# Zain-Jiang/Speech-Editing-Toolkit

Hardware: AMD Instinct MI355X
Metric: diffusion mel-frames/s (100-step p_sample, B=32/GPU, T=800) (higher is better)
Workload: dtype f32 (operands carried as 2 fp16 pieces, 3 MFMA products per term, fp32 accumulate: fp32-equivalent, see roofline.note)

## Files before the change

### include/set_amd.h

```cpp
#ifndef SET_AMD_H
#define SET_AMD_H

#include <stdint.h>

#ifdef __cplusplus
extern "C" {
#endif

#define SET_AMD_ABI_VERSION 5

#define SET_OK 0
#define SET_E_INVALID (-1)
#define SET_E_UNSUPPORTED (-2)
#define SET_E_LAUNCH (-3)

#define SET_ACT_NONE 0
#define SET_ACT_RELU 1
#define SET_ACT_GELU 2
#define SET_ACT_TANH 3
#define SET_ACT_SOFTPLUS 4
#define SET_ACT_MISH 5
#define SET_ACT_LRELU 6

#define SET_PRO_NONE 0
#define SET_PRO_LRELU 1
#define SET_PRO_DIV 2

#define SET_IMPL_NAIVE 1
#define SET_IMPL_MFMA 2
#define SET_IMPL_MFMA2 3

#define SET_IMPL_BF16 4
#define SET_IMPL_F16X2 5

#define SET_IMPL_FEWOUT 6

#define SET_DTYPE_F32 0
#define SET_DTYPE_BF16 1
#define SET_DTYPE_BF16_G16 2
#define SET_DTYPE_BF16_G16_X16 3

int set_abi_version(void);
const char *set_last_error(void);

typedef struct SetConv1dArgs {
    const float *in;
    const float *w;
    const float *bias;
    const float *res;
    const float *mask;
    const float *in_chan_add;
    float *out;
    int64_t in_bs, in_cs, out_bs, out_cs, res_bs, res_cs;
    int64_t w_base, w_sco, w_sci, w_stap;
    int32_t B, Cin, Cout, K, dil, pad;
    int32_t T_in, T_iter, T_out, out_stride, out_off;
    int32_t pro, act, accumulate, impl;
    float pro_param, act_param, alpha;
    float out_div;
} SetConv1dArgs;

int set_conv1d(const SetConv1dArgs *args, void *stream);

int64_t set_packed_conv_weight_size(int32_t Cout, int32_t Cin, int32_t K);
int set_pack_conv_weight(const float *w, float *wp, int32_t Cout, int32_t Cin, int32_t K,
                         int64_t w_base, int64_t w_sco, int64_t w_sci, int64_t w_stap, void *stream);

int64_t set_packed_conv_weight_x2_size(int32_t Cout, int32_t Cin, int32_t K);
int set_pack_conv_weight_x2(const float *w, void *wp, int32_t Cout, int32_t Cin, int32_t K, int64_t w_base, int64_t w_sco,
                            int64_t w_sci, int64_t w_stap, int32_t scale_exp, void *stream);
int64_t set_packed_conv_transpose_x2_size(int32_t Cout, int32_t Cin, int32_t k, int32_t u);
int set_pack_conv_transpose_x2(const float *w, void *wp, int32_t Cout, int32_t Cin, int32_t k, int32_t u, int32_t scale_exp,
                               void *stream);
int set_conv_transpose1d_x2(const float *in, const void *wp, const float *bias, float *out, int32_t B, int32_t Cin, int32_t Cout,
                            int32_t k, int32_t u, int32_t P, int32_t T_in, int32_t pro, float pro_param, void *stream);
int set_conv_x2_range_flag(int32_t *flag, int32_t reset);

typedef struct SetResblockPairArgs {
    const float *x;
    const void *w1;
    const float *b1;
    const void *w2;
    const float *b2;
    float *out;
    int64_t x_bs, x_cs, out_bs, out_cs;
    int32_t B, C, K, dil, T;
    int32_t accumulate;
    float slope, out_div;
} SetResblockPairArgs;
int64_t set_sizeof_resblock_pair_args(void);
int set_resblock_pair_x2_supported(int32_t C, int32_t K, int32_t dil, int32_t T);
int set_resblock_pair_x2(const SetResblockPairArgs *args, void *stream);

int64_t set_packed_conv_weight_v2_size(int32_t Cout, int32_t Cin, int32_t K);
int set_pack_conv_weight_v2(const float *w, float *wp, int32_t Cout, int32_t Cin, int32_t K, int32_t dil,
                            int64_t w_base, int64_t w_sco, int64_t w_sci, int64_t w_stap, void *stream);

int set_weight_norm_fold(const float *g, const float *v, float *w, int32_t n0, int64_t inner, void *stream);

int set_layernorm_ch(const float *x, const float *gamma, const float *beta, const float *mask, float *out,
                     int32_t B, int32_t C, int32_t T, float eps, void *stream);
int set_embedding_bct(const int64_t *idx, const float *table, float *out, int32_t B, int32_t T, int32_t C,
                      int32_t n_rows, float scale, int32_t accumulate, void *stream);
int set_embedding_bct_dev_scale(const int64_t *idx, const float *table, float *out, int32_t B, int32_t T, int32_t C,
                                int32_t n_rows, const float *scale_dev, int32_t accumulate, void *stream);
int set_abs_sum_mask(const float *x, float *mask, int32_t B, int32_t C, int32_t T, void *stream);
int set_index_mask(const int64_t *idx, float *mask, int64_t n, void *stream);
int set_expand_states(const float *enc, const int64_t *mel2ph, float *out, int32_t B, int32_t C,
                      int32_t T_txt, int32_t T, void *stream);
int set_add_chan_mask(const float *x, const float *add, const float *mask, float *out, int32_t B, int32_t C,
                      int32_t T, void *stream);
int set_masked_dur(const int64_t *mel2ph, const float *tmask, const int64_t *txt, int64_t *out, int32_t B,
                   int32_t T, int32_t T_txt, void *stream);
int set_pitch_coarse(const float *f0_in, const float *uv_in, const float *tmask, const int64_t *mel2ph_pad,
                     int32_t uv_from_logit, float *f0_denorm, int64_t *coarse, int64_t n, void *stream);
int set_transpose_btc_to_bct(const float *in, float *out, int32_t B, int32_t T, int32_t C, void *stream);
int set_transpose_bct_to_btc(const float *in, float *out, int32_t B, int32_t C, int32_t T, void *stream);
int set_sum_scale(const float *a, const float *b, const float *c, float *out, float div, int64_t n, void *stream);
int set_blend_mask(const float *a, const float *b, const float *m, float *out, int64_t n, int64_t inner, void *stream);
int set_mul_one_minus_mask(const float *x, const float *m, float *out, int64_t n, int64_t inner, void *stream);
int set_dur_total(const float *dur, const int64_t *txt, int64_t *total, int32_t B, int32_t T_txt, void *stream);
int set_length_regulate(const float *dur, const int64_t *txt, int64_t *mel2ph, int32_t B, int32_t T_txt,
                        int32_t T_out, void *stream);

int set_sinusoid_embed(const float *t, float *out, int32_t dim, int32_t n, void *stream);

int set_gate(const float *y, float *z, int32_t B, int32_t C, int32_t T, void *stream);
int set_res_skip(const float *x_in, const float *o, float *x_out, float *skip, int32_t B, int32_t C, int32_t T,
                 int32_t first, void *stream);

typedef struct SetDiffnetLayerArgs {
    const float *x_in;
    const float *condproj;
    const float *dstep;
    const float *w1p;
    const float *b_dil;
    const float *w2p;
    const float *b_out;
    float *x_out;
    float *skip;
    int64_t cp_bs, d_bs, d_cs;
    int32_t B, T, dil, first;
    uint64_t *dbg_clock;
} SetDiffnetLayerArgs;
int set_diffnet_layer(const SetDiffnetLayerArgs *args, void *stream);
int64_t set_diffnet_w1p_size(void);
int64_t set_diffnet_w2p_size(void);
int set_pack_diffnet_layer(const float *w_dil, const float *w_out, float *w1p, float *w2p, void *stream);
int set_pack_diffnet_layers(const float *w_dil, const float *w_out, int64_t wd_ls, int64_t wo_ls, float *w1p, float *w2p,
                            float *w1w, float *w2w, int32_t L, void *stream);

typedef struct SetDiffnetStackArgs {
    float *xa, *xb, *skip;
    const float *condproj;
    const float *dstep;
    const float *w1p_all;
    const float *w2p_all;
    const float *b_dil_all;
    const float *b_out_all;
    int32_t *sync_ws;
    int64_t cp_bs, cp_ls, d_bs, d_cs, d_ls;
    int32_t B, T, L, dilation_cycle_length;
    const float *w1w_all;
    const float *w2w_all;
    float *x_all;
    float *save_y;
    float *save_z;
    int32_t *err_flag;
    const float *w1s_all;
    const float *w2s_all;
    float *z_ws;
    const void *wx3_all;
    int32_t x3_mode;
} SetDiffnetStackArgs;
int set_diffnet_stack(const SetDiffnetStackArgs *args, void *stream);
int64_t set_sizeof_diffnet_stack_args(void);

int64_t set_diffnet_layer_x3_image_size(int32_t mode);
int set_pack_diffnet_layer_x3(const float *w_dil , const float *w_out , void *img, int32_t mode,
                              int32_t k1, int32_t k2, void *stream);
int set_diffnet_stack_variant(int B, int T, int dilation_cycle_length, int images);
int set_diffnet_stack_x3_winograd(int B, int T, int dilation_cycle_length, int images);
int64_t set_diffnet_w1w_size(void);
int set_pack_diffnet_layer_wino(const float *w_dil, const float *w_out, float *w1w, float *w2w, void *stream);

int set_posterior_step(const float *x0, const float *x_t, const float *eps, const float *coef4, int64_t coef_bs,
                       float *x_prev, int32_t B, int64_t per_batch, uint64_t seed, uint64_t offset, void *stream);
int set_q_sample(const float *x_start, const float *eps, const float *ab2, const float *nonpad, float *x_t,
                 int32_t B, int32_t M, int32_t T, void *stream);
int set_randn(float *out, int64_t n, uint64_t seed, uint64_t offset, void *stream);
int set_rng_seed_delta(const uint64_t *dev_word);
int set_stream_order(void *first, void *after, int32_t slot);
int set_stream_mark(void *stream, int32_t slot, int32_t dev);
int set_stream_mark_done(int32_t slot);
int set_stream_create_low_priority(void **out);

typedef struct SetDiffLoopArgs {
    int32_t B, T, M, L, steps, dilation_cycle_length;
    float *x;
    const float *noise;
    uint64_t seed;
    const float *condproj;
    const float *dstep;
    const float *coef4;
    const float *w_in_p;
    const float *b_in;
    const float *w1p_all;
    const float *w2p_all;
    const float *b_dil_all;
    const float *b_out_all;
    const float *w1w_all;
    const float *w2w_all;
    const float *w1s_all;
    const float *w2s_all;
    float *z_ws;
    const void *wx3_all;
    int32_t x3_mode;
    const void *w_skip_x2, *w_outp_x2, *w_in_x2;
    const float *w_skip_p;
    const float *b_skip;
    const float *w_outp_p;
    const float *b_outp;
    float *ws_x0, *ws_x1, *ws_skip, *ws_h;
    float *ws_x0pred;
    float *layer_span_ms;
    float *loop_ms;
    int32_t n_groups;
    int32_t persistent;
    int32_t *sync_ws;
    int32_t *err_flag;
    const float *cond;
    const void *img16_all;
    const float *b_cond_all;
    float *bf16_ws;
    int64_t bf16_ws_floats;
} SetDiffLoopArgs;
int set_diffusion_loop(const SetDiffLoopArgs *args, void *stream);

int set_conv1d_wgrad(const float *g, const float *x, const float *chan_add, float *dw, int32_t B, int32_t Cin,
                     int32_t Cout, int32_t K, int32_t dil, int32_t pad, int32_t T, int32_t T_in, int32_t pro,
                     float pro_param, int32_t impl, void *stream);

int64_t set_conv1d_wgrad_scratch_floats(int32_t B, int32_t Cin, int32_t Cout, int32_t K, int32_t T, int32_t dtype);
int set_conv1d_wgrad_det(const void *g, const void *x, const float *chan_add, float *dw, int32_t B, int32_t Cin,
                         int32_t Cout, int32_t K, int32_t dil, int32_t pad, int32_t T, int32_t T_in, int32_t pro,
                         float pro_param, int32_t dtype, float *scratch, int64_t scratch_floats, void *stream);
int64_t set_conv1d_wgrad_grouped_scratch_floats(int32_t groups, int32_t B, int32_t Cin, int32_t Cout, int32_t K, int32_t T);
int set_conv1d_wgrad_det_grouped(const void *g, const void *x, const float *chan_add, float *dw, int32_t groups, int64_t g_gs,
                                 int64_t x_gs, int64_t add_gs, int64_t dw_gs, int32_t B, int32_t Cin, int32_t Cout, int32_t K,
                                 int32_t dil, int32_t pad, int32_t T, int32_t T_in, int32_t dtype, float *scratch,
                                 int64_t scratch_floats, void *stream);

typedef struct SetDiffnetLayerBf16Args {
    const float *x_in;
    float *x_out;
    float *skip;
    const float *cond;
    const float *dstep;
    const void *img;
    const float *b_dil, *b_cond, *b_out;
    uint16_t *y16;
    uint16_t *z16;
    int64_t d_bs, d_cs;
    int32_t B, T, dil, first;
} SetDiffnetLayerBf16Args;
int64_t set_sizeof_diffnet_layer_bf16_args(void);
int64_t set_diffnet_layer_bf16_image_size(void);
int set_pack_diffnet_layer_bf16(const float *wdil , const float *wcond ,
                                const float *wout , void *img, void *stream);
int set_pack_diffnet_layers_bf16(const float *wdil, const float *wcond, const float *wout, int64_t sdil, int64_t scond, int64_t sout,
                                 void *img, int32_t L, void *stream);
int set_diffnet_layer_fwd_bf16(const SetDiffnetLayerBf16Args *args, void *stream);
typedef struct SetDiffnetLayersBf16Args {
    const float *x_in;
    float *x_out;
    float *skip;
    const float *cond;
    const float *dstep;
    const void *img;
    const float *b_dil, *b_cond, *b_out;
    float *scratch;
    int64_t scratch_floats;
    int64_t d_bs, d_cs, d_ls;
    int32_t B, T, l0, nl, dilation_cycle_length, first;
} SetDiffnetLayersBf16Args;
int64_t set_sizeof_diffnet_layers_bf16_args(void);
int64_t set_diffnet_layers_bf16_scratch_floats(int32_t B, int32_t T, int32_t l0, int32_t nl, int32_t dilation_cycle_length);
int32_t set_diffnet_layers_bf16_plan(int32_t B, int32_t T, int32_t L, int32_t dilation_cycle_length);
int set_diffnet_layers_fwd_bf16(const SetDiffnetLayersBf16Args *args, void *stream);
int set_debug_bf16_phase_buffer(uint64_t *buf);
int set_debug_split_phase_buffer(uint64_t *buf);
int set_debug_x3_phase_buffer(uint64_t *buf);
int set_debug_resblock_phase_buffer(uint64_t *buf);
int set_debug_conv_phase_buffer(uint64_t *buf);

typedef struct SetDiffnetLayerBf16BwdArgs {
    const float *dx_out;
    const float *dskip;
    const uint16_t *y16;
    const void *img;
    float *dx;
    uint16_t *dy16;
    uint16_t *do16;
    float *dcond;
    float *part_dbo;
    float *part_dby;
    float *part_dd;
    int32_t B, T, dil, dcond_first;
} SetDiffnetLayerBf16BwdArgs;
int64_t set_sizeof_diffnet_layer_bf16_bwd_args(void);
int32_t set_diffnet_layer_bwd_bf16_tiles(int32_t T, int32_t dil);
int set_diffnet_layer_bwd_bf16(const SetDiffnetLayerBf16BwdArgs *args, void *stream);
int set_diffnet_layer_bwd_reduce(const float *part_dbo, const float *part_dby, const float *part_dd, int32_t B, int32_t tiles,
                                 float *db_out, float *db_dil, float *db_cond, float *dd, int64_t dd_bs, void *stream);
int set_diffnet_layers_bwd_reduce(const float *part_dbo, const float *part_dby, const float *part_dd, int32_t B, int32_t tiles, int32_t L,
                                  float *db_out, int64_t s_out, float *db_dil, int64_t s_dil, float *db_cond, int64_t s_cond, float *dd,
                                  int64_t dd_bs, int64_t dd_ls, void *stream);
int set_partial_rows_sum(const float *part, float *out, int32_t groups, int32_t rows, int32_t cols, int32_t accumulate,
                         float scale, void *stream);

int set_step_proj_fwd(const float *h, const float *w, int64_t w_ls, const float *b, int64_t b_ls, float *out, int32_t L, int32_t C,
                      int32_t N, void *stream);
int64_t set_step_proj_bwd_scratch_floats(int32_t L, int32_t C, int32_t N);
int set_step_proj_bwd_dh(const float *g, const float *w, int64_t w_ls, float *dh, float *scratch, int32_t L, int32_t C, int32_t N,
                         void *stream);
int set_step_proj_bwd_dw(const float *h, const float *g, float *dw, int64_t dw_ls, float *db, int64_t db_ls, int32_t L, int32_t C,
                         int32_t N, void *stream);

int64_t set_packed_conv_weight_bf16_size(int32_t Cout, int32_t Cin, int32_t K);
int set_pack_conv_weight_bf16(const float *w, void *wp, int32_t Cout, int32_t Cin, int32_t K, int64_t w_base,
                              int64_t w_sco, int64_t w_sci, int64_t w_stap, void *stream);
#define SET_IMG_F32 0
#define SET_IMG_F32_BIG 1
#define SET_IMG_BF16 2
typedef struct SetPackDesc {
    const float *w;
    void *wp;
    int64_t w_base, w_sco, w_sci, w_stap, start;
    int32_t Cout, Cin, K, kind;
    int32_t CinP, CoutP, RB, ch_max;
} SetPackDesc;
int64_t set_sizeof_pack_desc(void);
int64_t set_fill_pack_desc(SetPackDesc *d, int32_t kind, int32_t dil);
int set_pack_conv_weights_batch(const SetPackDesc *descs_dev, int32_t n, int64_t total, void *stream);

int set_channel_sum_det(const float *x, float *out, int32_t B, int32_t C, int32_t T, float *scratch, void *stream);
int set_weighted_sum_det(const float *x, const float *w, float *out, int64_t n, int64_t inner, float *scratch, void *stream);
int set_sumsq_det(const float *g, float *out, int64_t n, float *scratch, void *stream);
int set_dur_loss_sums_det(const float *dur_pred, const int64_t *mel2ph, const int64_t *txt, const int64_t *word_id,
                          float *sums, int32_t B, int32_t T, int32_t T_txt, int32_t n_words, float *scratch, void *stream);
int set_pitch_loss_sums_det(const float *pp, const float *f0, const float *uv, const int64_t *mel2ph, float *sums,
                            int32_t B, int32_t T, float *scratch, void *stream);
int32_t set_scatter_rows_segments(int32_t T);
int set_scatter_rows_det(const int64_t *idx, const float *doutT, float *table, int32_t B, int32_t T, int32_t C,
                         int32_t n_rows, float scale, int32_t padding_idx, int32_t mode, float *scratch, void *stream);
int set_row_sum(const float *x, float *out, int64_t rows, int32_t T, float scale, void *stream);
int set_conv_epilogue_bwd(const float *dy, const float *y, const float *mask, float *g, int32_t B, int32_t C,
                          int32_t T, int32_t act, float alpha, void *stream);
int set_act_fwd(const float *z, float *y, int64_t n, int32_t act, float p, void *stream);
int set_act_bwd(const float *z, const float *dy, float *dz, int64_t n, int32_t act, float p, void *stream);
int set_act_bwd_scaled(const float *z, const float *dy, float *dz, int64_t n, int32_t act, float p, float scale, void *stream);
int set_gate_bwd(const float *y, const float *dz, float *dy, int32_t B, int32_t C, int32_t T, void *stream);
int set_res_skip_bwd(const float *dx_out, const float *dskip, float *dx, float *d_o, int32_t B, int32_t C, int32_t T,
                     void *stream);
int64_t set_layernorm_ch_bwd_scratch(int32_t B, int32_t C, int32_t T);
int set_layernorm_ch_bwd(const float *x, const float *gamma, const float *mask, const float *dy, float *dx,
                         float *dgamma, float *dbeta, float *partial, int32_t B, int32_t C, int32_t T, float eps,
                         void *stream);
int set_layernorm_ch_bwd_add(const float *x, const float *gamma, const float *mask, const float *dy, const float *add, float *dx,
                             float *dgamma, float *dbeta, float *partial, int32_t B, int32_t C, int32_t T, float eps, void *stream);
int set_dropout(const float *x, float *y, int64_t n, float p, uint64_t seed, uint64_t offset, void *stream);
int set_residual_dropout(const float *x, const float *z, const float *mask, float *y, int32_t B, int32_t C, int32_t T, float p,
                         uint64_t seed, uint64_t offset, void *stream);
int set_conv_epilogue_bwd_dropout(const float *dy, const float *mask, float *g2, float *gz, int32_t B, int32_t C, int32_t T, float p,
                                  uint64_t seed, uint64_t offset, void *stream);
int64_t set_stutter_head_scratch_floats(int32_t B, int32_t C, int32_t T);
int set_stutter_head_loss(const float *h, const float *w, const float *bias, const int64_t *labels, float *logits, float *stats,
                          float *scratch, int32_t B, int32_t C, int32_t T, void *stream);
int set_stutter_head_loss_bwd(const float *h, const float *w, const float *logits, const int64_t *labels, const float *stats,
                              const float *g_ce, const float *g_focal, float *dh, float *dw, float *db, float *scratch, int32_t B,
                              int32_t C, int32_t T, void *stream);
int set_stutter_head_bwd_reduce(const float *scratch, float *dw, float *db, int32_t B, int32_t C, int32_t T, void *stream);
int set_frame_weight(const float *target, float *w, int64_t frames, int32_t M, void *stream);
int set_l1_elem(const float *pred, const float *target, float *absd, float *sgn, int64_t n, void *stream);
int set_scale_bcast(const float *a, const float *w, float *out, int64_t n, int64_t inner, const float *scale_dev,
                    float scale, void *stream);
int set_ssim_filter(const float *img1, const float *img2, float bias, float *mu1, float *mu2, float *s11, float *s22,
                    float *s12, int32_t B, int32_t H, int32_t W, void *stream);
// ... 155 lines not shown
```

### speech-editing-toolkit_amd/_lib.py

```python
import ctypes as C
import os
import shutil
import subprocess

_PKG = os.path.dirname(os.path.abspath(__file__))
_ROOT = os.path.dirname(_PKG)
CSRC = os.path.join(_PKG, "csrc")
INCLUDE = os.path.join(_ROOT, "include")
LIB_PATH = os.path.join(_PKG, "libset_amd.so")
_LIB_OVERRIDE = os.environ.get("SET_AMD_LIB")
SOURCES = ["conv1d.hip", "weight_image.hip", "conv_x2.hip", "resblock_x2.hip", "glue.hip", "diffnet.hip", "diffnet_x3.hip", "boundary.hip", "diffusion_ops.hip", "diffusion_loop.hip",
           "train.hip", "attention.hip", "attention_fused.hip", "bf16.hip", "diffnet_bf16.hip", "stutter.hip", "melspec.hip", "mcd.hip", "stoi.hip", "wav_mcd.hip", "mel_loss.hip", "stft_loss.hip"]
HIPCC_FLAGS = ["--offload-arch=gfx950", "-O3", "-std=c++17", "-fPIC", "-shared", "-ffp-contract=off"]

OK, E_INVALID, E_UNSUPPORTED, E_LAUNCH = 0, -1, -2, -3
ACT = dict(none=0, relu=1, gelu=2, tanh=3, softplus=4, mish=5, lrelu=6)
PRO = dict(none=0, lrelu=1, div=2)
IMPL_NAIVE, IMPL_MFMA, IMPL_MFMA2, IMPL_BF16, IMPL_F16X2, IMPL_FEWOUT = 1, 2, 3, 4, 5, 6
DTYPE_F32, DTYPE_BF16, DTYPE_BF16_G16, DTYPE_BF16_G16_X16 = 0, 1, 2, 3

c_f32p = C.POINTER(C.c_float)
c_i64p = C.POINTER(C.c_int64)


class SetConv1dArgs(C.Structure):
    _fields_ = [
        ("inp", C.c_void_p), ("w", C.c_void_p), ("bias", C.c_void_p), ("res", C.c_void_p),
        ("mask", C.c_void_p), ("in_chan_add", C.c_void_p), ("out", C.c_void_p),
        ("in_bs", C.c_int64), ("in_cs", C.c_int64), ("out_bs", C.c_int64), ("out_cs", C.c_int64),
        ("res_bs", C.c_int64), ("res_cs", C.c_int64),
        ("w_base", C.c_int64), ("w_sco", C.c_int64), ("w_sci", C.c_int64), ("w_stap", C.c_int64),
        ("B", C.c_int32), ("Cin", C.c_int32), ("Cout", C.c_int32), ("K", C.c_int32), ("dil", C.c_int32),
        ("pad", C.c_int32),
        ("T_in", C.c_int32), ("T_iter", C.c_int32), ("T_out", C.c_int32), ("out_stride", C.c_int32),
        ("out_off", C.c_int32),
        ("pro", C.c_int32), ("act", C.c_int32), ("accumulate", C.c_int32), ("impl", C.c_int32),
        ("pro_param", C.c_float), ("act_param", C.c_float), ("alpha", C.c_float), ("out_div", C.c_float),
    ]


class SetDiffnetLayerArgs(C.Structure):
    _fields_ = [
        ("x_in", C.c_void_p), ("condproj", C.c_void_p), ("dstep", C.c_void_p), ("w1p", C.c_void_p),
        ("b_dil", C.c_void_p), ("w2p", C.c_void_p), ("b_out", C.c_void_p), ("x_out", C.c_void_p),
        ("skip", C.c_void_p),
        ("cp_bs", C.c_int64), ("d_bs", C.c_int64), ("d_cs", C.c_int64),
        ("B", C.c_int32), ("T", C.c_int32), ("dil", C.c_int32), ("first", C.c_int32),
        ("dbg_clock", C.c_void_p),
    ]


class SetDiffLoopArgs(C.Structure):
    _fields_ = [
        ("B", C.c_int32), ("T", C.c_int32), ("M", C.c_int32), ("L", C.c_int32), ("steps", C.c_int32),
        ("dilation_cycle_length", C.c_int32),
        ("x", C.c_void_p), ("noise", C.c_void_p), ("seed", C.c_uint64),
        ("condproj", C.c_void_p), ("dstep", C.c_void_p), ("coef4", C.c_void_p),
        ("w_in_p", C.c_void_p), ("b_in", C.c_void_p),
        ("w1p_all", C.c_void_p), ("w2p_all", C.c_void_p), ("b_dil_all", C.c_void_p), ("b_out_all", C.c_void_p),
        ("w1w_all", C.c_void_p), ("w2w_all", C.c_void_p),
        ("w1s_all", C.c_void_p), ("w2s_all", C.c_void_p), ("z_ws", C.c_void_p), ("wx3_all", C.c_void_p),
        ("x3_mode", C.c_int32),
        ("w_skip_x2", C.c_void_p), ("w_outp_x2", C.c_void_p), ("w_in_x2", C.c_void_p),
        ("w_skip_p", C.c_void_p), ("b_skip", C.c_void_p), ("w_outp_p", C.c_void_p), ("b_outp", C.c_void_p),
        ("ws_x0", C.c_void_p), ("ws_x1", C.c_void_p), ("ws_skip", C.c_void_p), ("ws_h", C.c_void_p),
        ("ws_x0pred", C.c_void_p),
        ("layer_span_ms", C.POINTER(C.c_float)),
        ("loop_ms", C.POINTER(C.c_float)),
        ("n_groups", C.c_int32),
        ("persistent", C.c_int32),
        ("sync_ws", C.c_void_p),
        ("err_flag", C.c_void_p),
        ("cond", C.c_void_p), ("img16_all", C.c_void_p), ("b_cond_all", C.c_void_p),
        ("bf16_ws", C.c_void_p), ("bf16_ws_floats", C.c_int64),
    ]


class SetDiffnetStackArgs(C.Structure):
    _fields_ = [
        ("xa", C.c_void_p), ("xb", C.c_void_p), ("skip", C.c_void_p), ("condproj", C.c_void_p), ("dstep", C.c_void_p),
        ("w1p_all", C.c_void_p), ("w2p_all", C.c_void_p), ("b_dil_all", C.c_void_p), ("b_out_all", C.c_void_p),
        ("sync_ws", C.c_void_p),
        ("cp_bs", C.c_int64), ("cp_ls", C.c_int64), ("d_bs", C.c_int64), ("d_cs", C.c_int64), ("d_ls", C.c_int64),
        ("B", C.c_int32), ("T", C.c_int32), ("L", C.c_int32), ("dilation_cycle_length", C.c_int32),
        ("w1w_all", C.c_void_p), ("w2w_all", C.c_void_p),
        ("x_all", C.c_void_p), ("save_y", C.c_void_p), ("save_z", C.c_void_p),
        ("err_flag", C.c_void_p),
        ("w1s_all", C.c_void_p), ("w2s_all", C.c_void_p), ("z_ws", C.c_void_p), ("wx3_all", C.c_void_p),
        ("x3_mode", C.c_int32),
    ]


class SetDiffnetLayerBf16Args(C.Structure):
    _fields_ = [
        ("x_in", C.c_void_p), ("x_out", C.c_void_p), ("skip", C.c_void_p), ("cond", C.c_void_p), ("dstep", C.c_void_p),
        ("img", C.c_void_p), ("b_dil", C.c_void_p), ("b_cond", C.c_void_p), ("b_out", C.c_void_p),
        ("y16", C.c_void_p), ("z16", C.c_void_p),
        ("d_bs", C.c_int64), ("d_cs", C.c_int64),
        ("B", C.c_int32), ("T", C.c_int32), ("dil", C.c_int32), ("first", C.c_int32),
    ]


class SetDiffnetLayersBf16Args(C.Structure):
    _fields_ = [
        ("x_in", C.c_void_p), ("x_out", C.c_void_p), ("skip", C.c_void_p), ("cond", C.c_void_p), ("dstep", C.c_void_p),
        ("img", C.c_void_p), ("b_dil", C.c_void_p), ("b_cond", C.c_void_p), ("b_out", C.c_void_p),
        ("scratch", C.c_void_p), ("scratch_floats", C.c_int64),
        ("d_bs", C.c_int64), ("d_cs", C.c_int64), ("d_ls", C.c_int64),
        ("B", C.c_int32), ("T", C.c_int32), ("l0", C.c_int32), ("nl", C.c_int32), ("dilation_cycle_length", C.c_int32),
        ("first", C.c_int32),
    ]


class SetDiffnetLayerBf16BwdArgs(C.Structure):
    _fields_ = [
        ("dx_out", C.c_void_p), ("dskip", C.c_void_p), ("y16", C.c_void_p), ("img", C.c_void_p),
        ("dx", C.c_void_p), ("dy16", C.c_void_p), ("do16", C.c_void_p), ("dcond", C.c_void_p),
        ("part_dbo", C.c_void_p), ("part_dby", C.c_void_p), ("part_dd", C.c_void_p),
        ("B", C.c_int32), ("T", C.c_int32), ("dil", C.c_int32), ("dcond_first", C.c_int32),
    ]


class SetResblockPairArgs(C.Structure):
    _fields_ = [
        ("x", C.c_void_p), ("w1", C.c_void_p), ("b1", C.c_void_p), ("w2", C.c_void_p), ("b2", C.c_void_p), ("out", C.c_void_p),
        ("x_bs", C.c_int64), ("x_cs", C.c_int64), ("out_bs", C.c_int64), ("out_cs", C.c_int64),
        ("B", C.c_int32), ("C", C.c_int32), ("K", C.c_int32), ("dil", C.c_int32), ("T", C.c_int32),
        ("accumulate", C.c_int32),
        ("slope", C.c_float), ("out_div", C.c_float),
    ]


IMG_F32, IMG_F32_BIG, IMG_BF16 = 0, 1, 2


class SetPackDesc(C.Structure):
    _fields_ = [
        ("w", C.c_void_p), ("wp", C.c_void_p),
        ("w_base", C.c_int64), ("w_sco", C.c_int64), ("w_sci", C.c_int64), ("w_stap", C.c_int64), ("start", C.c_int64),
        ("Cout", C.c_int32), ("Cin", C.c_int32), ("K", C.c_int32), ("kind", C.c_int32),
        ("CinP", C.c_int32), ("CoutP", C.c_int32), ("RB", C.c_int32), ("ch_max", C.c_int32),
    ]


class SetBmmArgs(C.Structure):
    _fields_ = [
        ("A", C.c_void_p), ("B", C.c_void_p), ("C", C.c_void_p),
        ("a_bo", C.c_int64), ("a_bi", C.c_int64), ("a_ms", C.c_int64), ("a_ks", C.c_int64),
        ("b_bo", C.c_int64), ("b_bi", C.c_int64), ("b_ks", C.c_int64), ("b_ns", C.c_int64),
        ("c_bo", C.c_int64), ("c_bi", C.c_int64), ("c_ms", C.c_int64), ("c_ns", C.c_int64),
        ("n_outer", C.c_int32), ("n_inner", C.c_int32), ("M", C.c_int32), ("N", C.c_int32), ("K", C.c_int32),
        ("alpha", C.c_float), ("accumulate", C.c_int32),
    ]


class SetAttnArgs(C.Structure):
    _fields_ = [
        ("q", C.c_void_p), ("k", C.c_void_p), ("v", C.c_void_p), ("o", C.c_void_p), ("lse", C.c_void_p), ("p", C.c_void_p),
        ("kpm", C.c_void_p),
        ("q_bs", C.c_int64), ("k_bs", C.c_int64), ("v_bs", C.c_int64), ("o_bs", C.c_int64),
        ("q_cs", C.c_int32), ("k_cs", C.c_int32), ("v_cs", C.c_int32), ("o_cs", C.c_int32),
        ("B", C.c_int32), ("heads", C.c_int32), ("head_dim", C.c_int32), ("Tq", C.c_int32), ("Tk", C.c_int32),
        ("scale", C.c_float), ("fill", C.c_float),
        ("bf16", C.c_int32),
    ]


class SetAttnBwdArgs(C.Structure):
    _fields_ = [
        ("fwd", SetAttnArgs),
        ("d_o", C.c_void_p), ("delta", C.c_void_p), ("dq", C.c_void_p), ("dk", C.c_void_p), ("dv", C.c_void_p),
        ("dq_bs", C.c_int64), ("dk_bs", C.c_int64), ("dv_bs", C.c_int64),
        ("dq_cs", C.c_int32), ("dk_cs", C.c_int32), ("dv_cs", C.c_int32),
    ]


class SetLogMelArgs(C.Structure):
    _fields_ = [
        ("wav", C.c_void_p), ("lengths", C.c_void_p), ("table", C.c_void_p), ("basis", C.c_void_p), ("mel", C.c_void_p),
        ("wav_bs", C.c_int64), ("log_scale", C.c_double),
        ("B", C.c_int32), ("N", C.c_int32), ("T", C.c_int32),
        ("n_fft", C.c_int32), ("hop", C.c_int32), ("n_mels", C.c_int32),
        ("bin_lo", C.c_int32), ("nbins", C.c_int32),
        ("pad", C.c_int32), ("reflect", C.c_int32), ("clamp_input", C.c_int32),
        ("mag_eps", C.c_float), ("floor", C.c_float), ("pad_", C.c_int32),
    ]


class SetMelLossFwdArgs(C.Structure):
    _fields_ = [
        ("mel_hat", C.c_void_p), ("mel_y", C.c_void_p), ("g_mel", C.c_void_p), ("log_hat", C.c_void_p), ("log_y", C.c_void_p),
        ("part", C.c_void_p), ("loss", C.c_void_p),
        ("log_scale", C.c_double),
        ("B", C.c_int32), ("T", C.c_int32), ("n_mels", C.c_int32),
        ("floor", C.c_float),
    ]


class SetMelLossBwdArgs(C.Structure):
    _fields_ = [
        ("wav", C.c_void_p), ("table", C.c_void_p), ("basis_t", C.c_void_p), ("itable", C.c_void_p), ("g_mel", C.c_void_p),
        ("spec", C.c_void_p), ("g_pad", C.c_void_p), ("g_wav", C.c_void_p),
        ("wav_bs", C.c_int64),
        ("B", C.c_int32), ("N", C.c_int32), ("T", C.c_int32),
        ("n_fft", C.c_int32), ("hop", C.c_int32), ("n_mels", C.c_int32),
        ("bin_lo", C.c_int32), ("nbins", C.c_int32), ("pad", C.c_int32),
        ("mag_eps", C.c_float), ("count", C.c_float), ("pad_", C.c_int32),
    ]


class SetStftLossArgs(C.Structure):
    _fields_ = [
        ("x", C.c_void_p), ("y", C.c_void_p), ("table", C.c_void_p), ("itable", C.c_void_p), ("u_sc", C.c_void_p), ("u_mag", C.c_void_p),
        ("g_m", C.c_void_p),
        ("mag", C.c_void_p), ("loss", C.c_void_p), ("spec", C.c_void_p), ("g_pad", C.c_void_p), ("g_wav", C.c_void_p),
        ("part", C.c_void_p), ("stats", C.c_void_p),
        ("x_bs", C.c_int64), ("y_bs", C.c_int64),
        ("B", C.c_int32), ("N", C.c_int32), ("T", C.c_int32),
        ("n_fft", C.c_int32), ("hop", C.c_int32), ("win", C.c_int32),
        ("which", C.c_int32), ("accumulate", C.c_int32),
        ("scale", C.c_float), ("pad_", C.c_int32),
    ]


_V, _I32, _I64, _U64, _F = C.c_void_p, C.c_int32, C.c_int64, C.c_uint64, C.c_float

SIGNATURES = {
    "set_abi_version": (C.c_int, []),
    "set_last_error": (C.c_char_p, []),
    "set_conv1d": (C.c_int, [C.POINTER(SetConv1dArgs), _V]),
    "set_packed_conv_weight_size": (_I64, [_I32, _I32, _I32]),
    "set_pack_conv_weight": (C.c_int, [_V, _V, _I32, _I32, _I32, _I64, _I64, _I64, _I64, _V]),
    "set_packed_conv_weight_v2_size": (_I64, [_I32, _I32, _I32]),
    "set_pack_conv_weight_v2": (C.c_int, [_V, _V, _I32, _I32, _I32, _I32, _I64, _I64, _I64, _I64, _V]),
    "set_weight_norm_fold": (C.c_int, [_V, _V, _V, _I32, _I64, _V]),
    "set_layernorm_ch": (C.c_int, [_V, _V, _V, _V, _V, _I32, _I32, _I32, _F, _V]),
    "set_embedding_bct": (C.c_int, [_V, _V, _V, _I32, _I32, _I32, _I32, _F, _I32, _V]),
    "set_embedding_bct_dev_scale": (C.c_int, [_V, _V, _V, _I32, _I32, _I32, _I32, _V, _I32, _V]),
    "set_abs_sum_mask": (C.c_int, [_V, _V, _I32, _I32, _I32, _V]),
    "set_index_mask": (C.c_int, [_V, _V, _I64, _V]),
    "set_expand_states": (C.c_int, [_V, _V, _V, _I32, _I32, _I32, _I32, _V]),
    "set_add_chan_mask": (C.c_int, [_V, _V, _V, _V, _I32, _I32, _I32, _V]),
# ... 260 lines not shown
```

### speech-editing-toolkit_amd/csrc/boundary.hip

```cpp
#include <stdlib.h>

#include "common.h"
#include "boundary_x2.h"
#include "diffnet_host.h"

namespace {
constexpr int DC = 256;
}

struct BoundaryArgs {
    const float *skip;
    float *x;
    const float *eps;
    const float *coef4;
    const float *w_skip_p, *b_skip, *w_outp_p, *b_outp, *w_in_p, *b_in;
    float *xin_next;
    float inv_div;
    float div;
    uint64_t seed, quad_offset;
    const uint64_t *seed_delta;
    int T, M, MP;
};
constexpr int BD_LD = 64;

__global__ void __launch_bounds__(256, 2) diffnet_boundary_kernel(BoundaryArgs a) {
    extern __shared__ __attribute__((aligned(16))) float smem[];
    const int tid = threadIdx.x, lane = tid & 63;
    const int w = __builtin_amdgcn_readfirstlane(tid >> 6);
    const int half = lane >> 5, l31 = lane & 31;
    const int b = blockIdx.y, t0 = blockIdx.x * 64, T = a.T, M = a.M;
    {
        const rsrc_t rs = make_rsrc(a.skip + (int64_t)b * DC * T);
        const unsigned vo = 4u * (unsigned)min(t0 + lane, T - 1);
        const bool tv = t0 + lane < T;
        for (int r0 = 0; r0 < 64; r0 += 16) {
            float v[16];
#pragma unroll
            for (int u = 0; u < 16; ++u) v[u] = buf_load(rs, vo, 4u * (unsigned)(64 * w + r0 + u) * (unsigned)T);
#pragma unroll
            for (int u = 0; u < 16; ++u) smem[(64 * w + r0 + u) * BD_LD + lane] = tv ? v[u] / a.div : 0.0f;
        }
    }
    __syncthreads();
    f32x16 acc[2][1][2];
#pragma unroll
    for (int i = 0; i < 2; ++i) {
        acc[i][0][0] = (f32x16){0};
        acc[i][0][1] = (f32x16){0};
        const float *wp = a.w_skip_p + (int64_t)(2 * w + i) * (DC / 2) * 64 + lane;
        const float *bp = smem + half * BD_LD + l31;
        gemm_groups<1, 2, 8>(acc[i], wp, bp, 2 * BD_LD, (DC / 2) / 8, [&](int) {
            wp += 8 * 64;
            bp += 8 * 2 * BD_LD;
        });
    }
    __syncthreads();
#pragma unroll
    for (int i = 0; i < 2; ++i)
#pragma unroll
        for (int r = 0; r < 16; ++r) {
            const int row = 32 * (2 * w + i) + mfma32_row(r, lane);
            const float bias = a.b_skip[row];
#pragma unroll
            for (int cb = 0; cb < 2; ++cb) smem[row * BD_LD + 32 * cb + l31] = fmaxf(acc[i][0][cb][r] + bias, 0.0f);
        }
    __syncthreads();
    const int rbn = (M + 31) / 32;
    f32x16 xo[1][2];
    xo[0][0] = (f32x16){0};
    xo[0][1] = (f32x16){0};
    if (w < rbn) {
        const float *wp = a.w_outp_p + (int64_t)w * (DC / 2) * 64 + lane;
        const float *bp = smem + half * BD_LD + l31;
        gemm_groups<1, 2, 8>(xo, wp, bp, 2 * BD_LD, (DC / 2) / 8, [&](int) {
            wp += 8 * 64;
            bp += 8 * 2 * BD_LD;
        });
    }
    __syncthreads();
    if (w < rbn) {
#pragma unroll
        for (int r = 0; r < 16; ++r) {
            const int row = 32 * w + mfma32_row(r, lane);
            const float bias = a.b_outp[min(row, M - 1)];
#pragma unroll
            for (int cb = 0; cb < 2; ++cb) smem[row * BD_LD + 32 * cb + l31] = row < M ? xo[0][cb][r] + bias : 0.0f;
        }
    }
    __syncthreads();
    {
        const float c1 = a.coef4[0], c2 = a.coef4[1], sig = a.coef4[3] * expf(0.5f * a.coef4[2]);
        uint64_t seed = a.seed;
        if (a.seed_delta) seed += *a.seed_delta;
        float *xb = a.x + (int64_t)b * M * T;
        const float *eb = a.eps ? a.eps + (int64_t)b * M * T : nullptr;
        for (int qi = tid; qi < a.MP * 16; qi += 256) {
            const int m = qi >> 4, tq = qi & 15, t = t0 + 4 * tq;
            float *cell = smem + m * BD_LD + 4 * tq;
            if (m < M && t < T) {
                const int64_t i = (int64_t)m * T + t;
                const f32x4 xt = *reinterpret_cast<const f32x4 *>(xb + i);
                float z[4];
                if (eb) {
                    const f32x4 e4 = *reinterpret_cast<const f32x4 *>(eb + i);
                    z[0] = e4[0]; z[1] = e4[1]; z[2] = e4[2]; z[3] = e4[3];
                } else {
                    randn4(seed, a.quad_offset + (uint64_t)(((int64_t)b * M * T + i) >> 2), z);
                }
                f32x4 o;
#pragma unroll
                for (int k = 0; k < 4; ++k) {
                    const float mean = c1 * cell[k] + c2 * xt[k];
                    o[k] = mean + sig * z[k];
                }
                *reinterpret_cast<f32x4 *>(xb + i) = o;
                *reinterpret_cast<f32x4 *>(cell) = o;
            } else {
                *reinterpret_cast<f32x4 *>(cell) = (f32x4){0.0f, 0.0f, 0.0f, 0.0f};
            }
        }
    }
    if (!a.xin_next) return;
    __syncthreads();
#pragma unroll
    for (int i = 0; i < 2; ++i) {
        acc[i][0][0] = (f32x16){0};
        acc[i][0][1] = (f32x16){0};
        const float *wp = a.w_in_p + (int64_t)(2 * w + i) * (a.MP / 2) * 64 + lane;
        const float *bp = smem + half * BD_LD + l31;
        gemm_groups<1, 2, 4>(acc[i], wp, bp, 2 * BD_LD, (a.MP / 2) / 4, [&](int) {
            wp += 4 * 64;
            bp += 4 * 2 * BD_LD;
        });
    }
    const rsrc_t ro = make_rsrc(a.xin_next + (int64_t)b * DC * T);
    float bin[2][16];
#pragma unroll
    for (int i = 0; i < 2; ++i)
#pragma unroll
        for (int r = 0; r < 16; ++r) bin[i][r] = (a.b_in + 32 * (2 * w + i) + urow16(r))[4 * half];
#pragma unroll
    for (int cb = 0; cb < 2; ++cb) {
        if (t0 + 32 * cb + l31 < T) {
            const unsigned so = 4u * (unsigned)(4 * half * T + t0 + 32 * cb + l31);
#pragma unroll
            for (int i = 0; i < 2; ++i)
#pragma unroll
                for (int r = 0; r < 16; ++r) {
                    const int ur = 32 * (2 * w + i) + urow16(r);
                    buf_store(fmaxf(acc[i][0][cb][r] + bin[i][r], 0.0f), ro, so, 4u * (unsigned)ur * (unsigned)T);
                }
        }
    }
}

struct BoundaryX2Args {
    BoundaryArgs g;
    const unsigned short *w_skip_x2, *w_outp_x2, *w_in_x2;
    int32_t *err_flag;
};

__global__ void __launch_bounds__(256, 2) diffnet_boundary_x2_kernel(BoundaryX2Args ax) {
    const BoundaryArgs &a = ax.g;
    extern __shared__ __attribute__((aligned(16))) unsigned char bl[];
    const int tid = threadIdx.x, lane = tid & 63;
    const int w = __builtin_amdgcn_readfirstlane(tid >> 6);
    const int half = lane >> 5, l31 = lane & 31;
    const int b = blockIdx.y, t0 = blockIdx.x * 64, T = a.T, M = a.M;
    const unsigned lane16 = 16u * (unsigned)lane;
    const unsigned T4 = 4u * (unsigned)T;
    float amax = 0.0f;
    {
        const int f = lane, cg = w;
        const rsrc_t rs = make_rsrc(a.skip + (int64_t)b * DC * T);
        const unsigned vo = 4u * (unsigned)min(t0 + f, T - 1);
        const bool tv = t0 + f < T;
        for (int c0 = 0; c0 < 64; c0 += 16) {
            float v[16];
#pragma unroll
            for (int u = 0; u < 16; ++u) v[u] = buf_load(rs, vo, (unsigned)(64 * cg + c0 + u) * T4);
#pragma unroll
            for (int q8 = 0; q8 < 2; ++q8) {
                u32x4_t u0, u1;
#pragma unroll
                for (int e = 0; e < 4; ++e) {
                    unsigned short p0[2], p1[2];
#pragma unroll
                    for (int k = 0; k < 2; ++k) {
                        const float sv = v[8 * q8 + 2 * e + k] / a.div;
                        const float x = tv ? sv : 0.0f;
                        amax = fmaxf(amax, fabsf(x));
                        bx_split(x, p0[k], p1[k]);
                    }
                    u0[e] = (unsigned)p0[0] | ((unsigned)p0[1] << 16);
                    u1[e] = (unsigned)p1[0] | ((unsigned)p1[1] << 16);
                }
                *reinterpret_cast<u32x4_t *>(bl + f * BX_XR + (64 * cg + c0 + 8 * q8) * 2) = u0;
                *reinterpret_cast<u32x4_t *>(bl + BX_PIECE + f * BX_XR + (64 * cg + c0 + 8 * q8) * 2) = u1;
            }
        }
    }
    __syncthreads();
    auto bfrag256 = [&](int ks, int cb) { return (unsigned)((cb * 32 + l31) * BX_XR + (ks * 16 + half * 8) * 2); };
    {
        const rsrc_t rw = make_rsrc(ax.w_skip_x2);
        const float inv = reinterpret_cast<const float *>(ax.w_skip_x2 + (DC / 32) * (DC / 16) * 1024)[1];
        f32x16 acc[2][2];
#pragma unroll
        for (int i = 0; i < 2; ++i)
#pragma unroll
            for (int cb = 0; cb < 2; ++cb) acc[i][cb] = (f32x16){0};
        bx_gemm<2>(acc, rw, lane16, 2 * w, DC / 16, DC / 16, bl, BX_PIECE, bfrag256);
        __syncthreads();
#pragma unroll
        for (int i = 0; i < 2; ++i)
#pragma unroll
            for (int cb = 0; cb < 2; ++cb)
#pragma unroll
                for (int g = 0; g < 4; ++g) {
                    unsigned short p0[4], p1[4];
#pragma unroll
                    for (int e = 0; e < 4; ++e) {
                        const int row = 32 * (2 * w + i) + 8 * g + 4 * half + e;
                        const float h = fmaxf(acc[i][cb][4 * g + e] * inv + a.b_skip[row], 0.0f);
                        amax = fmaxf(amax, h);
                        bx_split(h, p0[e], p1[e]);
                    }
                    const unsigned off = (unsigned)((cb * 32 + l31) * BX_XR + (32 * (2 * w + i) + 8 * g + 4 * half) * 2);
                    u32x2_t u;
                    u[0] = (unsigned)p0[0] | ((unsigned)p0[1] << 16); u[1] = (unsigned)p0[2] | ((unsigned)p0[3] << 16);
                    *reinterpret_cast<u32x2_t *>(bl + off) = u;
                    u[0] = (unsigned)p1[0] | ((unsigned)p1[1] << 16); u[1] = (unsigned)p1[2] | ((unsigned)p1[3] << 16);
                    *reinterpret_cast<u32x2_t *>(bl + BX_PIECE + off) = u;
                }
    }
    __syncthreads();
    float *xs = reinterpret_cast<float *>(bl);
    {
        const int rbn = (M + 31) / 32;
        f32x16 xo[1][2];
        xo[0][0] = (f32x16){0};
        xo[0][1] = (f32x16){0};
        const float inv = reinterpret_cast<const float *>(ax.w_outp_x2 + ((M + 31) / 32) * (DC / 16) * 1024)[1];
        if (w < rbn) bx_gemm<1>(xo, make_rsrc(ax.w_outp_x2), lane16, w, DC / 16, DC / 16, bl, BX_PIECE, bfrag256);
        __syncthreads();
        if (w < 3) {
#pragma unroll
            for (int r = 0; r < 16; ++r) {
                const int row = 32 * w + mfma32_row(r, lane);
                const float bias = a.b_outp[min(row, M - 1)];
#pragma unroll
                for (int cb = 0; cb < 2; ++cb) xs[row * 64 + 32 * cb + l31] = (w < rbn && row < M) ? xo[0][cb][r] * inv + bias : 0.0f;
            }
        }
    }
    __syncthreads();
    {
        const float c1 = a.coef4[0], c2 = a.coef4[1], sig = a.coef4[3] * expf(0.5f * a.coef4[2]);
        uint64_t seed = a.seed;
        if (a.seed_delta) seed += *a.seed_delta;
        float *xb = a.x + (int64_t)b * M * T;
        const float *eb = a.eps ? a.eps + (int64_t)b * M * T : nullptr;
        for (int qi = tid; qi < 96 * 16; qi += 256) {
            const int m = qi >> 4, tq = qi & 15, t = t0 + 4 * tq;
            float *cell = xs + m * 64 + 4 * tq;
            if (m < M && t < T) {
                const int64_t i = (int64_t)m * T + t;
                const f32x4 xt = *reinterpret_cast<const f32x4 *>(xb + i);
                float z[4];
                if (eb) {
                    const f32x4 e4 = *reinterpret_cast<const f32x4 *>(eb + i);
                    z[0] = e4[0]; z[1] = e4[1]; z[2] = e4[2]; z[3] = e4[3];
                } else {
                    randn4(seed, a.quad_offset + (uint64_t)(((int64_t)b * M * T + i) >> 2), z);
                }
                f32x4 o;
#pragma unroll
                for (int k = 0; k < 4; ++k) {
                    const float mean = c1 * cell[k] + c2 * xt[k];
                    o[k] = mean + sig * z[k];
                }
                *reinterpret_cast<f32x4 *>(xb + i) = o;
                *reinterpret_cast<f32x4 *>(cell) = o;
            } else {
                *reinterpret_cast<f32x4 *>(cell) = (f32x4){0.0f, 0.0f, 0.0f, 0.0f};
            }
        }
    }
    if (!a.xin_next) {
        if (!(amax < 32768.0f) && ax.err_flag) __hip_atomic_store(ax.err_flag, 2, __ATOMIC_RELAXED, __HIP_MEMORY_SCOPE_AGENT);
        return;
    }
    __syncthreads();
    unsigned char *xp = bl + BX_PIECE;
    constexpr unsigned XP_PIECE = 64 * BX_PR;
    {
        const int f = lane, cg = w;
#pragma unroll
        for (int q8 = 0; q8 < 3; ++q8) {
            u32x4_t u0, u1;
#pragma unroll
            for (int e = 0; e < 4; ++e) {
                unsigned short p0[2], p1[2];
#pragma unroll
                for (int k = 0; k < 2; ++k) {
                    const float x = xs[(24 * cg + 8 * q8 + 2 * e + k) * 64 + f];
                    amax = fmaxf(amax, fabsf(x));
                    bx_split(x, p0[k], p1[k]);
                }
                u0[e] = (unsigned)p0[0] | ((unsigned)p0[1] << 16);
                u1[e] = (unsigned)p1[0] | ((unsigned)p1[1] << 16);
            }
            *reinterpret_cast<u32x4_t *>(xp + f * BX_PR + (24 * cg + 8 * q8) * 2) = u0;
            *reinterpret_cast<u32x4_t *>(xp + XP_PIECE + f * BX_PR + (24 * cg + 8 * q8) * 2) = u1;
        }
    }
    if (!(amax < 32768.0f) && ax.err_flag) __hip_atomic_store(ax.err_flag, 2, __ATOMIC_RELAXED, __HIP_MEMORY_SCOPE_AGENT);
    __syncthreads();
    {
        const int ngin = ((M + 31) / 32) * 2;
        const float inv = reinterpret_cast<const float *>(ax.w_in_x2 + (DC / 32) * ngin * 1024)[1];
        f32x16 acc[2][2];
#pragma unroll
        for (int i = 0; i < 2; ++i)
#pragma unroll
            for (int cb = 0; cb < 2; ++cb) acc[i][cb] = (f32x16){0};
        bx_gemm<2>(acc, make_rsrc(ax.w_in_x2), lane16, 2 * w, ngin, ngin, xp, XP_PIECE,
                   [&](int ks, int cb) { return (unsigned)((cb * 32 + l31) * BX_PR + (ks * 16 + half * 8) * 2); });
        const rsrc_t ro = make_rsrc(a.xin_next + (int64_t)b * DC * T);
        float bin[2][16];
#pragma unroll
        for (int i = 0; i < 2; ++i)
#pragma unroll
            for (int r = 0; r < 16; ++r) bin[i][r] = (a.b_in + 32 * (2 * w + i) + urow16(r))[4 * half];
#pragma unroll
        for (int cb = 0; cb < 2; ++cb) {
            if (t0 + 32 * cb + l31 < T) {
                const unsigned so = 4u * (unsigned)(4 * half * T + t0 + 32 * cb + l31);
#pragma unroll
                for (int i = 0; i < 2; ++i)
#pragma unroll
                    for (int r = 0; r < 16; ++r) {
                        const int ur = 32 * (2 * w + i) + urow16(r);
                        buf_store(fmaxf(acc[i][cb][r] * inv + bin[i][r], 0.0f), ro, so, 4u * (unsigned)ur * (unsigned)T);
                    }
            }
        }
    }
}

bool boundary_fusable(const SetDiffLoopArgs &a) {
    if (const char *e = getenv("SET_AMD_FUSED_BOUNDARY"))
        if (atoi(e) == 0) return false;
    return a.T % 4 == 0 && a.M <= 96 && a.M >= 2 && ((a.M + 15) / 16 * 16 / 2) % 8 == 0;
}

int launch_boundary(const SetDiffLoopArgs &a, int Bg, const float *skip, float *x, const float *eps, int sid, uint64_t quad_offset,
                    float *xin_next, bool x2, hipStream_t s) {
    static SetDeviceOnce lds_once;
    if (int rc = set_lds_optin(lds_once, 80 * 1024, "boundary(attr)", diffnet_boundary_kernel, diffnet_boundary_x2_kernel)) return rc;
    BoundaryArgs g = {};
    g.skip = skip; g.x = x; g.eps = eps; g.coef4 = a.coef4 + 4 * sid;
    g.w_skip_p = a.w_skip_p; g.b_skip = a.b_skip; g.w_outp_p = a.w_outp_p; g.b_outp = a.b_outp;
    g.w_in_p = a.w_in_p; g.b_in = a.b_in; g.xin_next = xin_next;
    g.div = sqrtf((float)a.L); g.seed = a.seed; g.quad_offset = quad_offset; g.seed_delta = set_seed_delta_ptr();
    g.T = a.T; g.M = a.M; g.MP = (a.M + 15) / 16 * 16;
    if (x2) {
        BoundaryX2Args gx = {};
        gx.g = g;
        gx.w_skip_x2 = reinterpret_cast<const unsigned short *>(a.w_skip_x2);
        gx.w_outp_x2 = reinterpret_cast<const unsigned short *>(a.w_outp_x2);
        gx.w_in_x2 = reinterpret_cast<const unsigned short *>(a.w_in_x2);
        gx.err_flag = a.err_flag;
        hipLaunchKernelGGL(diffnet_boundary_x2_kernel, dim3((a.T + 63) / 64, Bg), dim3(256), (size_t)2 * BX_PIECE, s, gx);
    } else {
        hipLaunchKernelGGL(diffnet_boundary_kernel, dim3((a.T + 63) / 64, Bg), dim3(256), (size_t)DC * BD_LD * sizeof(float), s, g);
    }
    return set_check_launch("set_diffusion_loop(boundary)");
}
```

### speech-editing-toolkit_amd/csrc/common.h

```cpp
#pragma once
#include <hip/hip_runtime.h>
#include <stdint.h>
#include <stdio.h>

#include <atomic>
#include <type_traits>

#include "set_amd.h"

typedef float f32x16 __attribute__((ext_vector_type(16)));
typedef float f32x4 __attribute__((ext_vector_type(4)));
typedef unsigned u32x4_t __attribute__((ext_vector_type(4)));
typedef unsigned u32x2_t __attribute__((ext_vector_type(2)));
template <int N> using ic = std::integral_constant<int, N>;

extern thread_local char g_set_err[512];

static inline int set_fail(int code, const char *what, const char *detail) {
    snprintf(g_set_err, sizeof(g_set_err), "%s: %s", what, detail ? detail : "");
    return code;
}
static inline int set_check_launch(const char *what) {
    hipError_t e = hipGetLastError();
    if (e != hipSuccess) return set_fail(SET_E_LAUNCH, what, hipGetErrorString(e));
    return SET_OK;
}
#define SET_REQUIRE(cond, what)                                        \
    do {                                                               \
        if (!(cond)) return set_fail(SET_E_INVALID, what, #cond);      \
    } while (0)
#define SET_HIP(call, what)                                                        \
    do {                                                                           \
        hipError_t e__ = (call);                                                   \
        if (e__ != hipSuccess) return set_fail(SET_E_LAUNCH, what, hipGetErrorString(e__)); \
    } while (0)

struct SetDeviceOnce {
    std::atomic<uint64_t> done{0};
    template <typename F> int run(F &&f) {
        int dev = -1;
        const uint64_t bit = hipGetDevice(&dev) == hipSuccess && dev >= 0 && dev < 64 ? uint64_t(1) << dev : 0;
        if (done.load(std::memory_order_acquire) & bit) return SET_OK;
        const int rc = f();
        if (rc == SET_OK) done.fetch_or(bit, std::memory_order_release);
        return rc;
    }
};
template <typename... K>
static inline int set_lds_optin(SetDeviceOnce &once, int bytes, const char *what, K... kernels) {
    return once.run([&] {
        for (const void *k : {reinterpret_cast<const void *>(kernels)...})
            SET_HIP(hipFuncSetAttribute(k, hipFuncAttributeMaxDynamicSharedMemorySize, bytes), what);
        return SET_OK;
    });
}
static inline hipError_t set_cu_count(int *n_cu) {
    static std::atomic<int> cached[64];
    int dev = 0;
    hipError_t e = hipGetDevice(&dev);
    if (e != hipSuccess) return e;
    const bool slot = dev >= 0 && dev < 64;
    int n = slot ? cached[dev].load(std::memory_order_relaxed) : 0;
    if (n == 0) {
        e = hipDeviceGetAttribute(&n, hipDeviceAttributeMultiprocessorCount, dev);
        if (e != hipSuccess) return e;
        if (slot) cached[dev].store(n, std::memory_order_relaxed);
    }
    *n_cu = n;
    return hipSuccess;
}

const uint64_t *set_seed_delta_ptr();
static __global__ void __launch_bounds__(256) set_zero_words_kernel(unsigned *p, int64_t words) {
    const int64_t i = (int64_t)blockIdx.x * 256 + threadIdx.x;
    if (i < words) p[i] = 0u;
}
static inline bool set_aligned16(const void *a, const void *b, const void *c) {
    return ((reinterpret_cast<uintptr_t>(a) | reinterpret_cast<uintptr_t>(b) | reinterpret_cast<uintptr_t>(c)) & 15) == 0;
}
static inline hipError_t set_zero_async(void *p, size_t bytes, hipStream_t s) {
    const int64_t words = (int64_t)((bytes + 3) / 4);
    hipLaunchKernelGGL(set_zero_words_kernel, dim3((unsigned)((words + 255) / 256)), dim3(256), 0, s, reinterpret_cast<unsigned *>(p), words);
    return hipGetLastError();
}
static inline unsigned set_blocks(int64_t n, int per_block) { return (unsigned)((n + per_block - 1) / per_block); }
static inline int set_round_up(int x, int m) { return (x + m - 1) / m * m; }

__device__ __forceinline__ float dev_softplus(float x) { return x > 20.0f ? x : log1pf(expf(x)); }
__device__ __forceinline__ float dev_sigmoid(float x) { return 1.0f / (1.0f + expf(-x)); }

__device__ __forceinline__ float dev_act(float v, int act, float p) {
    switch (act) {
        case SET_ACT_RELU: return v > 0.0f ? v : 0.0f;
        case SET_ACT_GELU: return 0.5f * v * (1.0f + erff(v * 0.70710678118654752440f));
        case SET_ACT_TANH: return tanhf(v);
        case SET_ACT_SOFTPLUS: return dev_softplus(v);
        case SET_ACT_MISH: return v * tanhf(dev_softplus(v));
        case SET_ACT_LRELU: return v > 0.0f ? v : v * p;
        default: return v;
    }
}
__device__ __forceinline__ float dev_pro(float v, int pro, float p) {
    switch (pro) {
        case SET_PRO_LRELU: return v > 0.0f ? v : v * p;
        case SET_PRO_DIV: return v / p;
        default: return v;
    }
}
template <int PRO>
__device__ __forceinline__ float pro_c(float v, float p) {
    if constexpr (PRO == SET_PRO_LRELU) return v > 0.0f ? v : v * p;
    else if constexpr (PRO == SET_PRO_DIV) return v / p;
    else return v;
}
__device__ __forceinline__ float fsig(float x) { return __builtin_amdgcn_rcpf(1.0f + __expf(-x)); }
__device__ __forceinline__ float ftanh(float x) { return 1.0f - 2.0f * __builtin_amdgcn_rcpf(1.0f + __expf(2.0f * x)); }
__device__ __forceinline__ unsigned short f2bf(float x) { return __builtin_bit_cast(unsigned short, (__bf16)x); }
__device__ __forceinline__ float bf2f(unsigned short u) { return __builtin_bit_cast(float, (unsigned)u << 16); }
__device__ __forceinline__ unsigned short f2h(float x) { return __builtin_bit_cast(unsigned short, (_Float16)x); }
__device__ __forceinline__ float h2f(unsigned short u) { return (float)__builtin_bit_cast(_Float16, u); }

__device__ __forceinline__ float wave_sum(float v) {
#pragma unroll
    for (int o = 32; o > 0; o >>= 1) v += __shfl_xor(v, o);
    return v;
}

__device__ __forceinline__ int mfma32_row(int reg, int lane) { return (reg & 3) + 8 * (reg >> 2) + 4 * (lane >> 5); }
__device__ __forceinline__ int urow16(int r) { return (r & 3) + 8 * (r >> 2); }
__device__ __forceinline__ f32x16 mfma32(float a, float b, f32x16 c) {
    return __builtin_amdgcn_mfma_f32_32x32x2f32(a, b, c, 0, 0, 0);
}

__device__ __forceinline__ f32x16 mfma_f16(u32x4_t a, u32x4_t b, f32x16 c) {
    typedef _Float16 f16x8 __attribute__((ext_vector_type(8)));
    return __builtin_amdgcn_mfma_f32_32x32x16_f16(__builtin_bit_cast(f16x8, a), __builtin_bit_cast(f16x8, b), c, 0, 0, 0);
}
__device__ __forceinline__ f32x16 mfma_bf16(u32x4_t a, u32x4_t b, f32x16 c) {
    typedef __bf16 bf16x8 __attribute__((ext_vector_type(8)));
    return __builtin_amdgcn_mfma_f32_32x32x16_bf16(__builtin_bit_cast(bf16x8, a), __builtin_bit_cast(bf16x8, b), c, 0, 0, 0);
}

typedef __amdgpu_buffer_rsrc_t rsrc_t;
__device__ __forceinline__ rsrc_t make_rsrc(const void *p) {
    return __builtin_amdgcn_make_buffer_rsrc(const_cast<void *>(p), (short)0, (int)0x7fffffff, (int)0x00020000);
}
constexpr unsigned BUF_OOB = 0x80000000u;
__device__ __forceinline__ float buf_load(rsrc_t r, unsigned voff, unsigned soff) {
    return __builtin_bit_cast(float, __builtin_amdgcn_raw_buffer_load_b32(r, (int)voff, (int)soff, 0));
}
__device__ __forceinline__ f32x4 buf_load4(rsrc_t r, unsigned voff, unsigned soff) {
    return __builtin_bit_cast(f32x4, __builtin_amdgcn_raw_buffer_load_b128(r, (int)voff, (int)soff, 0));
}
__device__ __forceinline__ u32x4_t buf_load_u4(rsrc_t r, unsigned voff, unsigned soff) {
    return __builtin_amdgcn_raw_buffer_load_b128(r, (int)voff, (int)soff, 0);
}
__device__ __forceinline__ void buf_store4(f32x4 v, rsrc_t r, unsigned voff, unsigned soff) {
    __builtin_amdgcn_raw_buffer_store_b128(__builtin_bit_cast(u32x4_t, v), r, (int)voff, (int)soff, 0);
}
__device__ __forceinline__ void buf_store(float v, rsrc_t r, unsigned voff, unsigned soff) {
    __builtin_amdgcn_raw_buffer_store_b32(__builtin_bit_cast(unsigned, v), r, (int)voff, (int)soff, 0);
}
__device__ __forceinline__ f32x4 buf_load4_stream(rsrc_t r, unsigned voff, unsigned soff) {
    return __builtin_bit_cast(f32x4, __builtin_amdgcn_raw_buffer_load_b128(r, (int)voff, (int)soff, 2));
}
__device__ __forceinline__ void buf_store4_stream(f32x4 v, rsrc_t r, unsigned voff, unsigned soff) {
    __builtin_amdgcn_raw_buffer_store_b128(__builtin_bit_cast(u32x4_t, v), r, (int)voff, (int)soff, 16);
}
__device__ __forceinline__ void buf_atomic_add(float v, rsrc_t r, unsigned voff, unsigned soff) {
    (void)__builtin_amdgcn_raw_ptr_buffer_atomic_fadd_f32(v, r, (int)voff, (int)soff, 0);
}
__device__ __forceinline__ void buf_store_agent(float v, rsrc_t r, unsigned voff, unsigned soff) {
    __builtin_amdgcn_raw_buffer_store_b32(__builtin_bit_cast(unsigned, v), r, (int)voff, (int)soff, 16);
}

__device__ __forceinline__ void split2_f16(float a, float b, unsigned &p0, unsigned &p1) {
    typedef _Float16 h2_t __attribute__((ext_vector_type(2)));
    typedef float f2_t __attribute__((ext_vector_type(2)));
    const f2_t v = {a, b};
    const h2_t h0 = __builtin_convertvector(v, h2_t);
    const h2_t h1 = __builtin_convertvector(v - __builtin_convertvector(h0, f2_t), h2_t);
    p0 = __builtin_bit_cast(unsigned, h0);
    p1 = __builtin_bit_cast(unsigned, h1);
}

template <int RB> struct AVec;
template <> struct AVec<1> { typedef float type; };
template <> struct AVec<2> { typedef float type __attribute__((ext_vector_type(2))); };
template <> struct AVec<4> { typedef float type __attribute__((ext_vector_type(4))); };

template <int RB>
__device__ __forceinline__ float avec_get(const typename AVec<RB>::type &v, int r) {
    if constexpr (RB == 1) return v; else return v[r];
}

template <int RB, int NCB, int GS>
struct KOps {
    typename AVec<RB>::type A[GS];
    float B[GS][NCB];
};

template <int RB, int NCB, int GS, typename Adv>
__device__ __forceinline__ void gemm_groups(f32x16 (&acc)[RB][NCB], const typename AVec<RB>::type *&wp, const float *&bp,
                                            int rstep, int ng, Adv advance) {
    KOps<RB, NCB, GS> P, Q;
    auto load_step = [&](KOps<RB, NCB, GS> &o, int u) {
        o.A[u] = wp[u * 64];
#pragma unroll
        for (int cb = 0; cb < NCB; ++cb) o.B[u][cb] = bp[u * rstep + 32 * cb];
    };
    auto mma_step = [&](const KOps<RB, NCB, GS> &o, int u) {
        __builtin_amdgcn_s_setprio(1);
#pragma unroll
        for (int r = 0; r < RB; ++r)
#pragma unroll
            for (int cb = 0; cb < NCB; ++cb) acc[r][cb] = mfma32(avec_get<RB>(o.A[u], r), o.B[u][cb], acc[r][cb]);
        __builtin_amdgcn_s_setprio(0);
    };
#pragma unroll
    for (int u = 0; u < GS; ++u) load_step(P, u);
    for (int g = 0; g < ng; g += 2) {
        advance(g);
#pragma unroll
        for (int u = 0; u < GS; ++u) {
            load_step(Q, u);
            __builtin_amdgcn_sched_barrier(0);
            mma_step(P, u);
            __builtin_amdgcn_sched_barrier(0);
        }
        if (g + 2 < ng) advance(g + 1);
#pragma unroll
        for (int u = 0; u < GS; ++u) {
            load_step(P, u);
            __builtin_amdgcn_sched_barrier(0);
            mma_step(Q, u);
            __builtin_amdgcn_sched_barrier(0);
        }
    }
}
```

### speech-editing-toolkit_amd/csrc/diffnet_host.h

```cpp
#pragma once
#include "common.h"

enum StackFamily {
    STACK_DIRECT64 = 0,
    STACK_DIRECT32 = 1,
    STACK_WINO = 2,
    STACK_ROW_SPLIT = 3,
    STACK_X3_BF16 = 4,
    STACK_X3_F16 = 5,
};
constexpr int STACK_WINO_MAX_DIL = 8;

struct StackPlan {
    StackFamily family;
    bool split_x2;
    bool x3_wino;
    int x3_ncb;
    int n_cu;
    bool two_piece_fp16() const { return family == STACK_X3_F16 || (family == STACK_ROW_SPLIT && split_x2); }
};

int set_launch_diffnet_stack_f32(const SetDiffnetStackArgs &a, const StackPlan &p, hipStream_t s);
int set_launch_diffnet_stack_split_x2(const SetDiffnetStackArgs &a, const StackPlan &p, hipStream_t s);
int set_launch_diffnet_stack_x3(const SetDiffnetStackArgs &a, const StackPlan &p, hipStream_t s);

bool boundary_fusable(const SetDiffLoopArgs &a);
int launch_boundary(const SetDiffLoopArgs &a, int Bg, const float *skip, float *x, const float *eps, int sid, uint64_t quad_offset,
                    float *xin_next, bool x2, hipStream_t s);
```

### speech-editing-toolkit_amd/csrc/diffnet_x3.hip

```cpp
#include <stdio.h>
#include <stdlib.h>

#include "common.h"
#include "diffnet_host.h"
#include "phase_probe.h"
#include "stack_queue.h"

typedef __bf16 bf16x8_t __attribute__((ext_vector_type(8)));

SET_PHASE_PROBE_BUFFER(g_x3_phase_buf, set_debug_x3_phase_buffer)

namespace {

constexpr int XC = 256;
constexpr int X_MAXD = 8;
constexpr int XR = XC * 2 + 16;
constexpr int X_KS1 = 48;
constexpr int X_KS2 = 16;
constexpr float RSQRT2 = 0.70710678118654752440f;

__device__ __forceinline__ void split3(float a, unsigned short &p0, unsigned short &p1, unsigned short &p2) {
    p0 = f2bf(a);
    const float r1 = a - bf2f(p0);
    p1 = f2bf(r1);
// ... 390 lines not shown
    const bool first = a.first != 0;
    if constexpr (NU != 1) {
        if (!first) load_sk();
    }
#pragma unroll
    for (int cb = 0; cb < NCB; ++cb) {
        if (tv[cb]) {
            const rsrc_t rsk = make_rsrc(a.skp + ub[cb]);
#pragma unroll
            for (int u = 0; u < NU; ++u)
#pragma unroll
                for (int r = 0; r < 16; ++r)
                    buf_store_agent(first ? acc[u][1][cb][r] * is2 : acc[u][1][cb][r] * is2 + sk[u][cb][r], rsk, vo4[cb],
                                    (unsigned)(32 * (NU * w + u) + urow16(r)) * T4);
        }
    }
}

template <typename S, int NU, int NCB>
__global__ void __launch_bounds__(512 / NU, NU) diffnet_stack_x3_kernel(SetDiffnetStackArgs a, int tiles_per_utt, int ntiles, int ntasks,
                                                                        unsigned piece_bytes, int fault_tile) {
    extern __shared__ __attribute__((aligned(16))) unsigned char lds[];
    int *s_task = reinterpret_cast<int *>(lds + S::NP * piece_bytes + NCB * XC * sizeof(float));
    int *counter = a.sync_ws + SQ_COUNTER, *abort_flag = a.sync_ws + SQ_ABORT, *done = a.sync_ws + SQ_FLAGS;
    const int tid = threadIdx.x;
    PhaseProbe<13> pp;
    pp.start(g_x3_phase_buf && blockIdx.x == 0);
    if (tid == 0) s_task[0] = atomicAdd(counter, 1);
    __syncthreads();
    int n = __builtin_amdgcn_readfirstlane(s_task[0]);
    int i_done = -1, l_done = 0;
    while (n < ntasks) {
        const int l = n / ntiles, i = n - l * ntiles, j = i;
        X3Tile lt;
        stack_fill_x3_tile(lt, a, l, i, NCB, 1 << (l % a.dilation_cycle_length), x_nimg<S>());
        f32x16 acc[NU][2][NCB];
        if constexpr (NU == 1) x3_init<NU, NCB>(lt, acc);
        __builtin_amdgcn_sched_barrier(0);
        const int *f0 = done + i, *fl = done + (j > 0 ? i - 1 : i), *fr = done + (j < tiles_per_utt - 1 ? i + 1 : i);
        int peek = l, claimed = 0;
        if (tid == 0) {
            if (l > 0) peek = min(ld_agent(f0), min(ld_agent(fl), ld_agent(fr)));
            claimed = atomicAdd(counter, 1);
        }
        pp.lap(11);
        asm volatile("s_waitcnt vmcnt(0)" ::: "memory");
        pp.lap(12);
        if (tid == 0) {
            if (peek >= l) __builtin_amdgcn_fence(__ATOMIC_ACQUIRE, "agent");
            s_task[0] = claimed;
            s_task[1] = peek >= l ? 1 : 2;
        }
        __syncthreads();
        if (tid == 0 && i_done >= 0) stack_publish_store(done, i_done, l_done, fault_tile);
        i_done = -1;
        if (__builtin_amdgcn_readfirstlane(s_task[1]) == 2) {
            if (tid == 0) s_task[2] = stack_wait_tiles(f0, fl, fr, l, abort_flag, a.err_flag);
            __syncthreads();
            if (__builtin_amdgcn_readfirstlane(s_task[2]) == 0) break;
        }
        const int n_next = __builtin_amdgcn_readfirstlane(s_task[0]);
        x3_main<S, NU, NCB>(lt, acc, lds, piece_bytes, pp);
        i_done = i;
        l_done = l;
        n = n_next;
        pp.lap(5);
        pp.count(7);
    }
    asm volatile("s_waitcnt vmcnt(0)" ::: "memory");
    __syncthreads();
    if (tid == 0 && i_done >= 0) stack_publish_store(done, i_done, l_done, fault_tile);
    pp.flush(g_x3_phase_buf);
}

template <typename S, int NU, int NCB>
int launch_x3(const SetDiffnetStackArgs &a, int n_cu, hipStream_t s) {
    static SetDeviceOnce lds_once;
    if (int rc = set_lds_optin(lds_once, 160 * 1024, "set_diffnet_stack(x3 attr)", diffnet_stack_x3_kernel<S, NU, NCB>)) return rc;
    const int Q = a.B * ((a.T + 31) / 32);
    const int ntiles = (Q + NCB - 1) / NCB, tiles_per_utt = ntiles;
    const int64_t ntasks64 = (int64_t)ntiles * a.L;
    SET_REQUIRE(ntasks64 < (1ll << 30), "set_diffnet_stack(task count)");
    SET_REQUIRE((int64_t)2 * XC * a.T * 4 < ((int64_t)1 << 31), "set_diffnet_stack(split-operand kernel: T too large)");
    const int max_dil = 1 << (a.dilation_cycle_length - 1);
    const unsigned piece_bytes = (unsigned)(NCB * (32 + 2 * max_dil) * XR);
    const size_t ldsz = x3_lds_bytes<S, NCB>(max_dil);
    SET_HIP(set_zero_async(a.sync_ws, stack_sync_words(SQ_QUEUE, ntiles) * sizeof(int32_t), s), "set_diffnet_stack(memset)");
    const int grid = stack_grid(NU * n_cu, ntiles, ntasks64, true, 0);
    hipLaunchKernelGGL((diffnet_stack_x3_kernel<S, NU, NCB>), dim3(grid), dim3(512 / NU), ldsz, s, a, tiles_per_utt, ntiles, (int)ntasks64,
                       piece_bytes, stack_fault_tile());
    return set_check_launch("set_diffnet_stack");
}

typedef float f32x2 __attribute__((ext_vector_type(2)));
__device__ __forceinline__ f32x2 buf_load2(rsrc_t r, unsigned voff, unsigned soff) {
    return __builtin_bit_cast(f32x2, __builtin_amdgcn_raw_buffer_load_b64(r, (int)voff, (int)soff, 0));
}
__device__ __forceinline__ f32x2 buf_load2_nt(rsrc_t r, unsigned voff, unsigned soff) {
    return __builtin_bit_cast(f32x2, __builtin_amdgcn_raw_buffer_load_b64(r, (int)voff, (int)soff, X_NT));
}

constexpr int XRV = XC * 2 + 32;
template <int NB> constexpr unsigned xv_piece() { return 16 * NB * XRV; }
template <int NB> constexpr unsigned xv_plane() { return 2 * xv_piece<NB>(); }
template <int NB> constexpr unsigned xv_zpiece() { return 32 * NB * XR; }
template <int NB> constexpr unsigned xv_tile() { return 2 * xv_plane<NB>() > 2 * xv_zpiece<NB>() ? 2 * xv_plane<NB>() : 2 * xv_zpiece<NB>(); }
constexpr int XV_PF = 2;
constexpr int XV_PF2 = 2;
constexpr int X3V_FLAG_UNIT = 8;

__device__ __forceinline__ f32x4 mma16(u32x4_t a, u32x4_t b, f32x4 c) {
    return __builtin_amdgcn_mfma_f32_16x16x32_f16(__builtin_bit_cast(f16x8_t, a), __builtin_bit_cast(f16x8_t, b), c, 0, 0, 0);
}
__device__ __forceinline__ float row_prev(float v) {
    return __builtin_bit_cast(float, __builtin_amdgcn_update_dpp(0, __builtin_bit_cast(int, v), 0x111, 0xf, 0xf, false));
}
__device__ __forceinline__ float row_next(float v) {
    return __builtin_bit_cast(float, __builtin_amdgcn_update_dpp(0, __builtin_bit_cast(int, v), 0x101, 0xf, 0xf, false));
}

template <int NB>
__device__ __forceinline__ void x3v_init(const X3Tile &a, f32x4 (&PQ)[2][4][NB]) {
    typedef SplitF16x2 S;
    int tid = threadIdx.x;
    asm volatile("" : "+v"(tid));
    const int lane = tid & 63;
    const int w = __builtin_amdgcn_readfirstlane(tid >> 6);
    const int l15 = lane & 15, kg = lane >> 4;
    const int T = a.T;
    const unsigned T4 = 4u * (unsigned)T;
    const float hs = 0.5f * reinterpret_cast<const float *>(a.img + x_nimg<S>() - 8)[0];
    f32x4 bias[4];
#pragma unroll
    for (int mb = 0; mb < 4; ++mb) bias[mb] = *reinterpret_cast<const f32x4 *>(a.b_dil + (mb >= 2 ? XC : 0) + 32 * w + 16 * (mb & 1) + 4 * kg);
#pragma unroll
    for (int nb = 0; nb < NB; ++nb) {
        const X3Col c = x3_col(a, nb);
        const rsrc_t rcp = make_rsrc(a.cp + (int64_t)c.b * a.cp_bs);
        const unsigned vo = 4u * (unsigned)(4 * kg * T + min(c.t0 + 2 * l15, T - 2));
#pragma unroll
        for (int mb = 0; mb < 4; ++mb) {
            const unsigned row0 = (unsigned)((mb >= 2 ? XC : 0) + 32 * w + 16 * (mb & 1));
#pragma unroll
            for (int i = 0; i < 4; ++i) {
                const f32x2 v = buf_load2_nt(rcp, vo, (row0 + (unsigned)i) * T4);
                const float e = bias[mb][i] + v[0], o = bias[mb][i] + v[1];
                PQ[0][mb][nb][i] = hs * (e + o);
                PQ[1][mb][nb][i] = hs * (e - o);
            }
        }
    }
}

template <int NB, int PH>
__device__ __forceinline__ void x3v_stage_load(const X3Tile &a, int w, int lane, f32x2 (&x12)[NB][8], float (&xh)[NB][8]) {
    const int l15 = lane & 15, cs = lane >> 4;
    const int ch0 = 32 * w + 8 * cs;
    const int T = a.T;
    const unsigned T4 = 4u * (unsigned)T;
    const bool edge = l15 == 0 || l15 == 15;
#pragma unroll
    for (int nb = 0; nb < NB; ++nb) {
        const X3Col c = x3_col(a, nb);
        const rsrc_t rx = make_rsrc(a.xin + (int64_t)c.b * XC * T);
        const int t = c.t0 + 2 * l15;
        const unsigned vox = 4u * (unsigned)min(t, T - 2) + (unsigned)ch0 * T4;
#pragma unroll
        for (int k = 0; k < 8; ++k) x12[nb][k] = buf_load2(rx, vox, (unsigned)k * T4);
        if (PH == 1) {
            const int th = l15 == 0 ? c.t0 - 1 : c.t0 + 32;
            const unsigned voh = 4u * (unsigned)min(max(th, 0), T - 1) + (unsigned)ch0 * T4;
            if (edge) {
#pragma unroll
                for (int k = 0; k < 8; ++k) xh[nb][k] = buf_load(rx, voh, (unsigned)k * T4);
            }
        }
    }
}
template <int NB, int PH>
__device__ __forceinline__ float x3v_stage_store(const X3Tile &a, unsigned char *lds, const float *dsh, int w, int lane, const f32x2 (&x12)[NB][8],
                                                 const float (&xh)[NB][8]) {
    typedef SplitF16x2 S;
    const int l15 = lane & 15, cs = lane >> 4;
    const int ch0 = 32 * w + 8 * cs;
    const int T = a.T;
    const bool edge = l15 == 0 || l15 == 15;
    float amax = 0.0f;
#pragma unroll
    for (int nb = 0; nb < NB; ++nb) {
        const X3Col c = x3_col(a, nb);
        const int t = c.t0 + 2 * l15, th = l15 == 0 ? c.t0 - 1 : c.t0 + 32;
        const bool v12 = c.ok && t < T, vh = c.ok && edge && th >= 0 && th < T;
        const f32x4 dA = *reinterpret_cast<const f32x4 *>(dsh + nb * XC + ch0);
        const f32x4 dB = *reinterpret_cast<const f32x4 *>(dsh + nb * XC + ch0 + 4);
        u32x4_t u[2][2];
#pragma unroll
        for (int e2 = 0; e2 < 4; ++e2) {
            float V[2][2];
#pragma unroll
            for (int h = 0; h < 2; ++h) {
                const int e = 2 * e2 + h;
                const float ds = e < 4 ? dA[e & 3] : dB[e & 3];
                const float d1 = v12 ? x12[nb][e][0] + ds : 0.0f, d2 = v12 ? x12[nb][e][1] + ds : 0.0f;
                if (PH == 0) {
                    V[0][h] = d1 + d2;
                    V[1][h] = d2 - d1;
                } else {
                    float d0 = row_prev(d2), d3 = row_next(d1);
                    const float hv = vh ? xh[nb][e] + ds : 0.0f;
                    d0 = l15 == 0 ? hv : d0;
                    d3 = l15 == 15 ? hv : d3;
                    V[0][h] = d0 - d2;
                    V[1][h] = d1 - d3;
                }
            }
#pragma unroll
            for (int j = 0; j < 2; ++j) {
                amax = fmaxf(fmaxf(amax, fabsf(V[j][0])), fabsf(V[j][1]));
                unsigned pw[2];
                S::split2(V[j][0], V[j][1], pw);
                u[j][0][e2] = pw[0];
                u[j][1][e2] = pw[1];
            }
        }
#pragma unroll
        for (int j = 0; j < 2; ++j)
#pragma unroll
            for (int q = 0; q < 2; ++q) *reinterpret_cast<u32x4_t *>(lds + j * xv_plane<NB>() + q * xv_piece<NB>() + (16 * nb + l15) * XRV + ch0 * 2) = u[j][q];
    }
    return amax;
}

template <int NB, int PFV>
__device__ __forceinline__ void x3v_plane(f32x4 (&acc)[4][NB], u32x4_t (&A)[PFV][4][2], rsrc_t img, unsigned lane16, unsigned abase, int seg,
                                          const unsigned char *bplane, unsigned boff) {
    typedef SplitF16x2 S;
    const int ks_last = 16 * (seg >> 1) + 15;
    for (int kb = 0; kb < 8; kb += PFV) {
#pragma unroll
        for (int p = 0; p < PFV; ++p) {
            const int kc = kb + p, ks = 8 * seg + kc;
            u32x4_t Bv[NB][2];
#pragma unroll
            for (int nb = 0; nb < NB; ++nb)
#pragma unroll
                for (int q = 0; q < 2; ++q) Bv[nb][q] = *reinterpret_cast<const u32x4_t *>(bplane + q * xv_piece<NB>() + boff + (unsigned)(nb * 16 * XRV) + (unsigned)kc * 64u);
            __builtin_amdgcn_sched_barrier(0);
            __builtin_amdgcn_s_setprio(1);
#pragma unroll
            for (int t = 0; t < S::NPROD; ++t)
#pragma unroll
                for (int mb = 0; mb < 4; ++mb)
#pragma unroll
                    for (int nb = 0; nb < NB; ++nb) acc[mb][nb] = mma16(A[p][mb][S::qa(t)], Bv[nb][S::qb(t)], acc[mb][nb]);
            __builtin_amdgcn_s_setprio(0);
            const int kn = min(ks + PFV, ks_last);
#pragma unroll
            for (int mb = 0; mb < 4; ++mb)
#pragma unroll
                for (int q = 0; q < 2; ++q) A[p][mb][q] = buf_load_u4(img, lane16, abase + (unsigned)(((kn * 4 + mb) * 2 + q) * 1024));
            __builtin_amdgcn_sched_barrier(0);
        }
    }
}

template <int NB>
__device__ __forceinline__ void x3v_main(const X3Tile &a, f32x4 (&PQ)[2][4][NB], unsigned char *lds, PhaseProbe<11> &pp, PhaseTimeline<32> &tl) {
    pp.lap(0); tl.mark(8);
    typedef SplitF16x2 S;
    constexpr int PFV = XV_PF;
    int tid = threadIdx.x;
    asm volatile("" : "+v"(tid));
    const int lane = tid & 63;
    const int w = __builtin_amdgcn_readfirstlane(tid >> 6);
    const int l15 = lane & 15, kg = lane >> 4;
    const int half = lane >> 5, l31 = lane & 31;
    const int T = a.T;
    const unsigned T4 = 4u * (unsigned)T;
    const unsigned lane16 = 16u * (unsigned)lane;
    float *dsh = reinterpret_cast<float *>(lds + xv_tile<NB>());
    const rsrc_t rw = make_rsrc(a.img);
    const float *sc = reinterpret_cast<const float *>(a.img + x_n1<S>() + x_n2<S>());
    const float s2 = sc[2], is2 = sc[3];
    const float is1w = reinterpret_cast<const float *>(a.img + x_nimg<S>() - 8)[1];
    const float cg2 = is1w * -1.4426950408889634f, cf2 = is1w * 2.8853900817779268f;
    const unsigned abase = (unsigned)((x_n1<S>() + x_n2<S>() + 8) * 2) + (unsigned)(w * X_KSV * 4 * 2 * 1024);
    const unsigned boff = (unsigned)(l15 * XRV + kg * 16);
    u32x4_t A[PFV][4][2];
    f32x2 x12[NB][8];
    float xh[NB][8];
    x3v_stage_load<NB, 0>(a, w, lane, x12, xh);
    float amax = x3v_stage_store<NB, 0>(a, lds, dsh, w, lane, x12, xh);
#pragma unroll
    for (int p = 0; p < PFV; ++p)
#pragma unroll
        for (int mb = 0; mb < 4; ++mb)
#pragma unroll
            for (int q = 0; q < 2; ++q) A[p][mb][q] = buf_load_u4(rw, lane16, abase + (unsigned)(((p * 4 + mb) * 2 + q) * 1024));
    tl.mark(20);
    __syncthreads();
    pp.lap(1); tl.mark(9);
    x3v_plane<NB, PFV>(PQ[0], A, rw, lane16, abase, 0, lds, boff);
    x3v_plane<NB, PFV>(PQ[1], A, rw, lane16, abase, 1, lds + xv_plane<NB>(), boff);
    pp.lap(2); tl.mark(10);
    x3v_stage_load<NB, 1>(a, w, lane, x12, xh);
    __builtin_amdgcn_sched_barrier(0);
#pragma unroll
    for (int mb = 0; mb < 4; ++mb)
#pragma unroll
        for (int nb = 0; nb < NB; ++nb)
#pragma unroll
            for (int i = 0; i < 4; ++i) {
                const float pp = PQ[0][mb][nb][i], qq = PQ[1][mb][nb][i];
                PQ[0][mb][nb][i] = pp + qq;
                PQ[1][mb][nb][i] = pp - qq;
            }
    __syncthreads();
    tl.mark(21);
    amax = fmaxf(amax, x3v_stage_store<NB, 1>(a, lds, dsh, w, lane, x12, xh));
    if (!(amax < 32768.0f) && a.err_flag) __hip_atomic_store(a.err_flag, 2, __ATOMIC_RELAXED, __HIP_MEMORY_SCOPE_AGENT);
#pragma unroll
    for (int p = 0; p < PFV; ++p)
#pragma unroll
        for (int mb = 0; mb < 4; ++mb)
#pragma unroll
            for (int q = 0; q < 2; ++q) A[p][mb][q] = buf_load_u4(rw, lane16, abase + (unsigned)((((16 + p) * 4 + mb) * 2 + q) * 1024));
    tl.mark(22);
    __syncthreads();
    pp.lap(3); tl.mark(11);
    x3v_plane<NB, PFV>(PQ[0], A, rw, lane16, abase, 2, lds, boff);
    x3v_plane<NB, PFV>(PQ[1], A, rw, lane16, abase, 3, lds + xv_plane<NB>(), boff);
    pp.lap(4); tl.mark(12);
    bool tv[NB];
    unsigned vo4[NB];
    int64_t ub[NB];
#pragma unroll
    for (int cb = 0; cb < NB; ++cb) {
        const X3Col c = x3_col(a, cb);
        const int t = c.t0 + l31;
        tv[cb] = c.ok && t < T;
        vo4[cb] = 4u * (unsigned)(4 * half * T + min(t, T - 1));
        ub[cb] = (int64_t)c.b * XC * T;
    }
    float xres[NB][16];
#pragma unroll
    for (int cb = 0; cb < NB; ++cb) {
        const rsrc_t rx = make_rsrc(a.xin + ub[cb]);
#pragma unroll
        for (int r = 0; r < 16; ++r) xres[cb][r] = buf_load(rx, vo4[cb], (unsigned)(32 * w + urow16(r)) * T4);
    }
    __syncthreads();
    tl.mark(23);
#pragma unroll
    for (int nb = 0; nb < NB; ++nb) {
        const X3Col c = x3_col(a, nb);
        const bool tvp = c.ok && c.t0 + 2 * l15 < T;
#pragma unroll
        for (int eo = 0; eo < 2; ++eo)
#pragma unroll
            for (int m = 0; m < 2; ++m) {
                float zz[4];
#pragma unroll
                for (int i = 0; i < 4; ++i) {
                    const float u = __builtin_amdgcn_exp2f(PQ[eo][m][nb][i] * cg2);
                    const float v = __builtin_amdgcn_exp2f(fminf(PQ[eo][m + 2][nb][i] * cf2, 64.0f));
                    const float g = (v - 1.0f) * __builtin_amdgcn_rcpf((1.0f + u) * (1.0f + v));
                    zz[i] = tvp ? g : 0.0f;
                }
                unsigned plo[2], phi[2];
                S::split2(zz[0], zz[1], plo);
                S::split2(zz[2], zz[3], phi);
                const unsigned off = (unsigned)((32 * nb + 2 * l15 + eo) * XR + (32 * w + 16 * m + 4 * kg) * 2);
#pragma unroll
                for (int q = 0; q < 2; ++q) {
                    u32x2_t uu;
                    uu[0] = plo[q];
                    uu[1] = phi[q];
                    *reinterpret_cast<u32x2_t *>(lds + q * xv_zpiece<NB>() + off) = uu;
                }
            }
    }
    f32x16 acc[1][2][NB];
#pragma unroll
    for (int rb = 0; rb < 2; ++rb) {
        const float *bo = a.b_out + (rb ? XC : 0) + 32 * w;
#pragma unroll
        for (int r = 0; r < 16; ++r) {
            const float blo = bo[urow16(r)], bhi = bo[urow16(r) + 4];
            const float bias = half ? bhi : blo;
#pragma unroll
            for (int cb = 0; cb < NB; ++cb) acc[0][rb][cb][r] = (rb == 0 ? bias + xres[cb][r] : bias) * s2;
        }
    }
    tl.mark(24);
    __syncthreads();
    pp.lap(8); tl.mark(16);
    gemm_x3<S, X_KS2, 1, NB, XV_PF2>(acc, rw, lane16, (unsigned)(x_n1<S>() * 2 + w * X_KS2 * 2 * 2 * 1024), (unsigned)(X_KS2 * 2 * 2 * 1024), lds,
                                     xv_zpiece<NB>(), [&](int ks, int cb) { return (unsigned)((cb * 32 + l31) * XR + (ks * 16 + half * 8) * 2); });
    pp.lap(9); tl.mark(17);
    const bool first = a.first != 0;
    float sk[NB][16];
    if (!first) {
#pragma unroll
        for (int cb = 0; cb < NB; ++cb) {
            const rsrc_t rsk = make_rsrc(a.skp + ub[cb]);
#pragma unroll
            for (int r = 0; r < 16; ++r) sk[cb][r] = buf_load_nt(rsk, vo4[cb], (unsigned)(32 * w + urow16(r)) * T4);
        }
    }
#pragma unroll
    for (int cb = 0; cb < NB; ++cb) {
        if (tv[cb]) {
            const rsrc_t rxo = make_rsrc(a.xout + ub[cb]);
#pragma unroll
            for (int r = 0; r < 16; ++r) buf_store_agent((acc[0][0][cb][r] * is2) * RSQRT2, rxo, vo4[cb], (unsigned)(32 * w + urow16(r)) * T4);
        }
    }
    tl.mark(25);
#pragma unroll
    for (int cb = 0; cb < NB; ++cb) {
        if (tv[cb]) {
            const rsrc_t rsk = make_rsrc(a.skp + ub[cb]);
#pragma unroll
            for (int r = 0; r < 16; ++r)
                buf_store_agent(first ? acc[0][1][cb][r] * is2 : acc[0][1][cb][r] * is2 + sk[cb][r], rsk, vo4[cb], (unsigned)(32 * w + urow16(r)) * T4);
        }
    }
    pp.lap(10); tl.mark(18);
}

#ifndef X3V_TL_TASK
#define X3V_TL_TASK 10
#endif
template <int NB>
__global__ void __launch_bounds__(512, 1) diffnet_stack_x3v_kernel(SetDiffnetStackArgs a, int ntiles, int ntasks, int fault_tile) {
    typedef SplitF16x2 S;
    extern __shared__ __attribute__((aligned(16))) unsigned char lds[];
    int *s_task = reinterpret_cast<int *>(lds + xv_tile<NB>() + NB * XC * sizeof(float));
    int *counter = a.sync_ws + SQ_COUNTER, *abort_flag = a.sync_ws + SQ_ABORT, *done = a.sync_ws + SQ_FLAGS;
    const int tid = threadIdx.x;
    PhaseProbe<11> pp;
    pp.start(SET_PHASE_PROBE == 1 && g_x3_phase_buf && blockIdx.x == 0);
    PhaseTimeline<32> tl;
    if (tid == 0) s_task[0] = atomicAdd(counter, 1);
    __syncthreads();
    int n = __builtin_amdgcn_readfirstlane(s_task[0]);
    int i_done = -1, l_done = 0;
#if SET_PHASE_PROBE == 2
    int n_mine = 0;
#endif
    while (n < ntasks) {
        const int l = n / ntiles, i = n - l * ntiles;
        X3Tile lt;
        stack_fill_x3_tile(lt, a, l, i, NB, 1, x_nimg<S>());
        f32x4 PQ[2][4][NB];
        tl.mark(0);
        if (i_done >= 0) {
            asm volatile("s_waitcnt vmcnt(0)" ::: "memory");
            if ((tid & 63) == 0) stack_publish_add(done, i_done, l_done, fault_tile);
            i_done = -1;
        }
        __builtin_amdgcn_sched_barrier(0);
        float dsv[(NB * XC + 511) / 512];
#pragma unroll
        for (int j = 0; j < (NB * XC + 511) / 512; ++j) {
            const int idx = min(tid + 512 * j, NB * XC - 1);
            dsv[j] = lt.dstep[(int64_t)x3_col(lt, idx >> 8).b * lt.d_bs + (int64_t)(idx & (XC - 1)) * lt.d_cs];
        }
        x3v_init<NB>(lt, PQ);
        __builtin_amdgcn_sched_barrier(0);
        const int *f0 = done + i, *fl = done + (i > 0 ? i - 1 : i), *fr = done + (i < ntiles - 1 ? i + 1 : i);
        int peek = l, claimed = 0;
        if (tid == 0) {
            if (l > 0) peek = min(ld_agent(f0), min(ld_agent(fl), ld_agent(fr))) / X3V_FLAG_UNIT;
            claimed = atomicAdd(counter, 1);
        }
        tl.mark(1);
        asm volatile("s_waitcnt vmcnt(0)" ::: "memory");
        tl.mark(2);
        {
            float *dsh = reinterpret_cast<float *>(lds + xv_tile<NB>());
#pragma unroll
            for (int j = 0; j < (NB * XC + 511) / 512; ++j)
                if (tid + 512 * j < NB * XC) dsh[tid + 512 * j] = dsv[j];
        }
        if (tid == 0) {
            if (peek >= l) __builtin_amdgcn_fence(__ATOMIC_ACQUIRE, "agent");
            s_task[0] = claimed;
            s_task[1] = peek >= l ? 1 : 2;
        }
        __syncthreads();
        tl.mark(3);
        if (__builtin_amdgcn_readfirstlane(s_task[1]) == 2) {
            if (tid == 0) s_task[2] = stack_wait_tiles(f0, fl, fr, l * X3V_FLAG_UNIT, abort_flag, a.err_flag);
            __syncthreads();
            if (__builtin_amdgcn_readfirstlane(s_task[2]) == 0) break;
        }
        const int n_next = __builtin_amdgcn_readfirstlane(s_task[0]);
        tl.mark(4);
        x3v_main<NB>(lt, PQ, lds, pp, tl);
#if SET_PHASE_PROBE == 2
        if (++n_mine == X3V_TL_TASK && (tid == 0 || tid == 448) && g_x3_phase_buf) {
            const rsrc_t rt = make_rsrc(g_x3_phase_buf);
            const unsigned row = (unsigned)(2 * blockIdx.x + (tid ? 1 : 0)) * 128u;
#pragma unroll
            for (int k = 0; k < 32; ++k) __builtin_amdgcn_raw_buffer_store_b32((unsigned)(tl.ts[k] - tl.ts[0]), rt, (int)(row + 4 * k), 0, 0);
            __builtin_amdgcn_raw_buffer_store_b32((unsigned)n, rt, (int)(row + 20), 0, 0);
            __builtin_amdgcn_raw_buffer_store_b32((unsigned)s_task[1], rt, (int)(row + 24), 0, 0);
            __builtin_amdgcn_raw_buffer_store_b32((unsigned)tl.ts[0], rt, (int)(row + 28), 0, 0);
        } else if (n_mine == X3V_TL_TASK + 1 && (tid == 0 || tid == 448) && g_x3_phase_buf) {
            __builtin_amdgcn_raw_buffer_store_b32((unsigned)tl.ts[0], make_rsrc(g_x3_phase_buf), (int)((unsigned)(2 * blockIdx.x + (tid ? 1 : 0)) * 128u + 124u), 0, 0);
        }
#endif
        i_done = i;
        l_done = l;
        n = n_next;
        pp.lap(5);
        pp.count(7);
    }
    asm volatile("s_waitcnt vmcnt(0)" ::: "memory");
    if ((tid & 63) == 0 && i_done >= 0) stack_publish_add(done, i_done, l_done, fault_tile);
    pp.flush(g_x3_phase_buf);
}

template <int NB>
int launch_x3v(const SetDiffnetStackArgs &a, int n_cu, hipStream_t s) {
    static SetDeviceOnce lds_once;
    if (int rc = set_lds_optin(lds_once, 160 * 1024, "set_diffnet_stack(x3v attr)", diffnet_stack_x3v_kernel<NB>)) return rc;
    const int Q = a.B * ((a.T + 31) / 32);
    const int ntiles = (Q + NB - 1) / NB;
    const int64_t ntasks64 = (int64_t)ntiles * a.L;
    SET_REQUIRE(ntasks64 < (1ll << 30), "set_diffnet_stack(task count)");
    SET_REQUIRE((int64_t)2 * XC * a.T * 4 < ((int64_t)1 << 31), "set_diffnet_stack(split-operand kernel: T too large)");
    SET_REQUIRE(a.dilation_cycle_length == 1 && a.T % 2 == 0, "set_diffnet_stack(x3v: dilation 1 and even T only)");
    const size_t ldsz = (size_t)xv_tile<NB>() + NB * XC * sizeof(float) + 16;
    SET_HIP(set_zero_async(a.sync_ws, stack_sync_words(SQ_QUEUE, ntiles) * sizeof(int32_t), s), "set_diffnet_stack(memset)");
    const int grid = stack_grid(n_cu, ntiles, ntasks64, NB == 2, 0);
    hipLaunchKernelGGL(diffnet_stack_x3v_kernel<NB>, dim3(grid), dim3(512), ldsz, s, a, ntiles, (int)ntasks64, stack_fault_tile());
    return set_check_launch("set_diffnet_stack");
}


constexpr int SX_PF = 8;

__device__ __forceinline__ float buf_load_sc1(rsrc_t r, unsigned voff, unsigned soff) {
    return __builtin_bit_cast(float, __builtin_amdgcn_raw_buffer_load_b32(r, (int)voff, (int)soff, 16));
}
__device__ __forceinline__ u32x4_t buf_load_u4_sc1(rsrc_t r, unsigned voff, unsigned soff) {
    return __builtin_amdgcn_raw_buffer_load_b128(r, (int)voff, (int)soff, 16);
}

template <int NKS, typename BF>
__device__ __forceinline__ void sx_gemm(f32x16 &acc, u32x4_t (&A)[SX_PF][2], rsrc_t img, unsigned lane16, unsigned abase,
                                        const unsigned char *lds, unsigned piece_bytes, BF bfrag) {
    unsigned bo = bfrag(0);
    u32x4_t b0 = *reinterpret_cast<const u32x4_t *>(lds + bo);
    u32x4_t b1 = *reinterpret_cast<const u32x4_t *>(lds + piece_bytes + bo);
#pragma unroll 1
    for (int kb = 0; kb < NKS; kb += SX_PF) {
#pragma unroll
        for (int p = 0; p < SX_PF; ++p) {
            const int ks = kb + p;
            const unsigned bn = bfrag(min(ks + 1, NKS - 1));
            const u32x4_t nb0 = *reinterpret_cast<const u32x4_t *>(lds + bn);
            const u32x4_t nb1 = *reinterpret_cast<const u32x4_t *>(lds + piece_bytes + bn);
            acc = SplitF16x2::mma(A[p][1], b0, acc);
            acc = SplitF16x2::mma(A[p][0], b1, acc);
            acc = SplitF16x2::mma(A[p][0], b0, acc);
            const int kn = min(ks + SX_PF, NKS - 1);
            A[p][0] = buf_load_u4(img, lane16, abase + (unsigned)(kn * 4 * 1024));
            A[p][1] = buf_load_u4(img, lane16, abase + (unsigned)((kn * 4 + 1) * 1024));
            b0 = nb0;
            b1 = nb1;
            __builtin_amdgcn_sched_barrier(0);
        }
    }
}
__device__ __forceinline__ void sx_preload(u32x4_t (&A)[SX_PF][2], rsrc_t img, unsigned lane16, unsigned abase) {
#pragma unroll
    for (int p = 0; p < SX_PF; ++p) {
        A[p][0] = buf_load_u4(img, lane16, abase + (unsigned)(p * 4 * 1024));
        A[p][1] = buf_load_u4(img, lane16, abase + (unsigned)((p * 4 + 1) * 1024));
    }
}

__global__ void __launch_bounds__(256, 1) diffnet_stack_split_x2_kernel(SetDiffnetStackArgs a, int tiles_per_utt, int ntiles,
                                                                         unsigned piece_bytes, int fault_tile, int nofence) {
    typedef SplitF16x2 S;
    extern __shared__ __attribute__((aligned(16))) unsigned char lds[];
    float *gs = reinterpret_cast<float *>(lds + 2 * piece_bytes);
    float *dsh = gs + 64 * 32;
    int *s_ok = reinterpret_cast<int *>(dsh + XC);
    int *abort_flag = a.sync_ws + SQ_ABORT, *ready = a.sync_ws + SQ_FLAGS, *zcnt = a.sync_ws + sq_flags2(ntiles);
    const int tid = threadIdx.x, lane = tid & 63, half = lane >> 5, l31 = lane & 31;
    const int j = __builtin_amdgcn_readfirstlane(tid >> 6);
    if ((int)blockIdx.x >= 4 * ntiles) {
        const int hp = blockIdx.x & 3;
        for (int l = 1; l < a.L; ++l) {
            if (l >= 2 && !stack_wait_pace(ready, 4 * (l - 1), abort_flag)) return;
            const unsigned char *img = reinterpret_cast<const unsigned char *>(a.wx3_all) + (int64_t)l * x_nimg<S>() * 2;
            const rsrc_t r1 = make_rsrc(img + (size_t)(2 * hp) * X_KS1 * 4 * 1024);
            const rsrc_t r2 = make_rsrc(img + x_n1<S>() * 2 + (size_t)(2 * hp) * X_KS2 * 4 * 1024);
            for (unsigned off = 16u * tid; off < 2u * X_KS1 * 4 * 1024; off += 8u * 4096u) {
#pragma unroll
                for (unsigned q = 0; q < 8; ++q) {
                    const u32x4_t v = buf_load_u4(r1, off + q * 4096u, 0u);
                    asm volatile("" ::"v"(v));
                }
            }
            for (unsigned off = 16u * tid; off < 2u * X_KS2 * 4 * 1024; off += 8u * 4096u) {
#pragma unroll
                for (unsigned q = 0; q < 8; ++q) {
                    const u32x4_t v = buf_load_u4(r2, off + q * 4096u, 0u);
                    asm volatile("" ::"v"(v));
                }
            }
        }
        return;
    }
    const int i = blockIdx.x >> 2, h = blockIdx.x & 3;
    const int b = i / tiles_per_utt, jt = i - b * tiles_per_utt;
    const int T = a.T, t0 = jt * 32;
    const int il = jt > 0 ? i - 1 : i, ir = jt < tiles_per_utt - 1 ? i + 1 : i;
    const unsigned T4 = 4u * (unsigned)T;
    const int w8 = 2 * h + (j & 1), rb = j >> 1;
    const int ch0 = 32 * w8;
    const int tq = t0 + l31;
    const bool tv = tq < T;
    const unsigned vo4 = 4u * (unsigned)(4 * half * T + min(tq, T - 1));
    const unsigned lane16 = 16u * (unsigned)lane;
    unsigned short *zt = reinterpret_cast<unsigned short *>(a.z_ws) + (int64_t)i * (2 * 32 * XC);
    const rsrc_t rz = make_rsrc(zt);
    const rsrc_t rsk = make_rsrc(a.skip + (int64_t)b * XC * T);
    PhaseProbe<8> pp;
    pp.start(g_x3_phase_buf && blockIdx.x == 5);
    for (int l = 0; l < a.L; ++l) {
        const int d = 1 << (l % a.dilation_cycle_length);
        const unsigned short *img = reinterpret_cast<const unsigned short *>(a.wx3_all) + (int64_t)l * x_nimg<S>();
        const rsrc_t rw = make_rsrc(img);
        const float *sc = reinterpret_cast<const float *>(img + x_n1<S>() + x_n2<S>());
        const float s1 = sc[0], is1 = sc[1], s2 = sc[2], is2 = sc[3];
        const rsrc_t rxin = make_rsrc(((l & 1) ? a.xb : a.xa) + (int64_t)b * XC * T);
        const rsrc_t rxout = make_rsrc(((l & 1) ? a.xa : a.xb) + (int64_t)b * XC * T);
        const rsrc_t rcp = make_rsrc(a.condproj + (int64_t)l * a.cp_ls + (int64_t)b * a.cp_bs);
        const float *dstep = a.dstep + (int64_t)l * a.d_ls + (int64_t)b * a.d_bs;
        const float *bd = a.b_dil_all + (int64_t)l * 512 + rb * XC + ch0, *bo = a.b_out_all + (int64_t)l * 512 + rb * XC + ch0;
        u32x4_t A[SX_PF][2];
        const unsigned ab1 = (unsigned)(((w8 * X_KS1) * 2 + rb) * 2 * 1024);
        sx_preload(A, rw, lane16, ab1);
        f32x16 acc;
#pragma unroll
        for (int r = 0; r < 16; ++r) {
            const float blo = bd[urow16(r)], bhi = bd[urow16(r) + 4];
            acc[r] = (half ? bhi : blo) + buf_load(rcp, vo4, (unsigned)(rb * XC + ch0 + urow16(r)) * T4);
        }
        if (tid == 0) *s_ok = l == 0 ? 1 : stack_wait_parts(ready + i, ready + il, ready + ir, 4 * l, abort_flag, a.err_flag, !nofence);
        __syncthreads();
        if (__builtin_amdgcn_readfirstlane(*s_ok) == 0) return;
        pp.lap(0);
        {
            const int f = tid & 31, cg = tid >> 5;
            dsh[tid] = dstep[(int64_t)tid * a.d_cs];
            float amax = 0.0f;
            auto put = [&](int row, const float (&v)[32], bool valid) {
#pragma unroll
                for (int q8 = 0; q8 < 4; ++q8) {
                    unsigned short p[8][2];
                    const f32x4 d0 = *reinterpret_cast<const f32x4 *>(dsh + 32 * cg + 8 * q8);
                    const f32x4 d1 = *reinterpret_cast<const f32x4 *>(dsh + 32 * cg + 8 * q8 + 4);
#pragma unroll
                    for (int e = 0; e < 8; ++e) {
                        const float xs = v[8 * q8 + e] + (e < 4 ? d0[e & 3] : d1[e & 3]);
                        const float xv = valid ? xs : 0.0f;
                        amax = fmaxf(amax, fabsf(xv));
                        S::split(xv, p[e]);
                    }
                    u32x4_t u[2];
                    pack8<2>(p, u);
                    *reinterpret_cast<u32x4_t *>(lds + row * XR + (32 * cg + 8 * q8) * 2) = u[0];
                    *reinterpret_cast<u32x4_t *>(lds + piece_bytes + row * XR + (32 * cg + 8 * q8) * 2) = u[1];
                }
            };
            const int t = t0 - d + f, th = t0 - d + 32 + f;
            const bool tvx = t >= 0 && t < T, has_h = f < 2 * d, tvh = th >= 0 && th < T;
            const unsigned vox = 4u * (unsigned)min(max(t, 0), T - 1), voh = 4u * (unsigned)min(max(th, 0), T - 1);
            float vx[32], vh[32];
            if (nofence) {
#pragma unroll
                for (int k = 0; k < 32; ++k) vx[k] = buf_load_sc1(rxin, vox, (unsigned)(32 * cg + k) * T4);
                if (has_h) {
#pragma unroll
                    for (int k = 0; k < 32; ++k) vh[k] = buf_load_sc1(rxin, voh, (unsigned)(32 * cg + k) * T4);
                }
            } else {
#pragma unroll
                for (int k = 0; k < 32; ++k) vx[k] = buf_load(rxin, vox, (unsigned)(32 * cg + k) * T4);
                if (has_h) {
#pragma unroll
                    for (int k = 0; k < 32; ++k) vh[k] = buf_load(rxin, voh, (unsigned)(32 * cg + k) * T4);
                }
            }
            __syncthreads();
            put(f, vx, tvx);
            if (has_h) put(32 + f, vh, tvh);
            if (!(amax < 32768.0f) && a.err_flag) __hip_atomic_store(a.err_flag, 2, __ATOMIC_RELAXED, __HIP_MEMORY_SCOPE_AGENT);
        }
#pragma unroll
        for (int r = 0; r < 16; ++r) acc[r] *= s1;
        __syncthreads();
        pp.lap(1);
        sx_gemm<X_KS1>(acc, A, rw, lane16, ab1, lds, piece_bytes, [&](int ks) {
            return (unsigned)((l31 + (ks >> 4) * d) * XR + ((ks & 15) * 16 + half * 8) * 2);
        });
        pp.lap(2);
        if (rb == 1) {
#pragma unroll
            for (int r = 0; r < 16; ++r) gs[(32 * (j & 1) + urow16(r) + 4 * half) * 32 + l31] = ftanh(acc[r] * is1);
        }
        __syncthreads();
        if (rb == 0) {
#pragma unroll
            for (int g = 0; g < 4; ++g) {
                unsigned short p[4][2];
#pragma unroll
                for (int e = 0; e < 4; ++e) {
                    const int r = 4 * g + e;
                    const float zz = fsig(acc[r] * is1) * gs[(32 * (j & 1) + urow16(r) + 4 * half) * 32 + l31];
                    S::split(tv ? zz : 0.0f, p[e]);
                }
                const unsigned off = (unsigned)(l31 * (XC * 2) + (ch0 + 8 * g + 4 * half) * 2);
#pragma unroll
                for (int q = 0; q < 2; ++q) {
                    u32x2_t u;
                    u[0] = (unsigned)p[0][q] | ((unsigned)p[1][q] << 16);
                    u[1] = (unsigned)p[2][q] | ((unsigned)p[3][q] << 16);
                    __builtin_amdgcn_raw_buffer_store_b64(u, rz, (int)(off + (unsigned)q * (32u * XC * 2u)), 0, 16);
                }
            }
        }
        asm volatile("s_waitcnt vmcnt(0)" ::: "memory");
        __syncthreads();
        if (tid == 0) stack_publish_add(zcnt, i, l, fault_tile, false);
        pp.lap(3);
        const unsigned ab2 = (unsigned)(x_n1<S>() * 2 + ((w8 * X_KS2) * 2 + rb) * 2 * 1024);
        sx_preload(A, rw, lane16, ab2);
        float prev[16];
        {
            const rsrc_t rp = make_rsrc(rb == 0 ? ((l & 1) ? a.xb : a.xa) + (int64_t)b * XC * T : a.skip + (int64_t)b * XC * T);
#pragma unroll
            for (int r = 0; r < 16; ++r) prev[r] = buf_load(rp, vo4, (unsigned)(ch0 + urow16(r)) * T4);
        }
#pragma unroll
        for (int r = 0; r < 16; ++r) {
            const float blo = bo[urow16(r)], bhi = bo[urow16(r) + 4];
            const float bias = half ? bhi : blo;
            acc[r] = (rb == 0 ? bias + prev[r] : bias) * s2;
        }
        if (tid == 0) *s_ok = stack_wait_parts(zcnt + i, zcnt + i, zcnt + i, 4 * (l + 1), abort_flag, a.err_flag, !nofence);
        __syncthreads();
        if (__builtin_amdgcn_readfirstlane(*s_ok) == 0) return;
        pp.lap(4);
        {
            u32x4_t zv[8];
#pragma unroll
            for (int k = 0; k < 8; ++k)
                zv[k] = nofence ? buf_load_u4_sc1(rz, 16u * (unsigned)tid, 4096u * (unsigned)k) : buf_load_u4(rz, 16u * (unsigned)tid, 4096u * (unsigned)k);
#pragma unroll
            for (int k = 0; k < 8; ++k) {
                const int unit = tid + 256 * k;
                const int q = unit >> 10, fr = (unit >> 5) & 31, part = unit & 31;
                *reinterpret_cast<u32x4_t *>(lds + q * piece_bytes + fr * XR + part * 16) = zv[k];
            }
        }
        __syncthreads();
        pp.lap(5);
        sx_gemm<X_KS2>(acc, A, rw, lane16, ab2, lds, piece_bytes, [&](int ks) {
            return (unsigned)(l31 * XR + (ks * 16 + half * 8) * 2);
        });
        pp.lap(6);
        if (tv && rb == 0) {
#pragma unroll
            for (int r = 0; r < 16; ++r) buf_store_agent((acc[r] * is2) * RSQRT2, rxout, vo4, (unsigned)(ch0 + urow16(r)) * T4);
        } else if (tv) {
            const bool first = l == 0;
#pragma unroll
            for (int r = 0; r < 16; ++r)
                buf_store(first ? acc[r] * is2 : acc[r] * is2 + prev[r], rsk, vo4, (unsigned)(ch0 + urow16(r)) * T4);
        }
        asm volatile("s_waitcnt vmcnt(0)" ::: "memory");
        __syncthreads();
        if (tid == 0) stack_publish_add(ready, i, l, fault_tile, h == 0);
        pp.lap(7);
    }
    pp.flush(g_x3_phase_buf);
}

}

int set_launch_diffnet_stack_split_x2(const SetDiffnetStackArgs &a, const StackPlan &p, hipStream_t s) {
    static SetDeviceOnce lds_once;
    if (int rc = set_lds_optin(lds_once, 80 * 1024, "set_diffnet_stack(split x2 attr)", diffnet_stack_split_x2_kernel)) return rc;
    const int tiles = (a.T + 31) / 32, nt = a.B * tiles;
    const int max_dil = 1 << (a.dilation_cycle_length - 1);
    const unsigned piece_bytes = (unsigned)((32 + 2 * max_dil) * XR);
    const size_t ldsz = (size_t)2 * piece_bytes + (64 * 32 + XC) * sizeof(float) + 16;
    SET_HIP(set_zero_async(a.sync_ws, stack_sync_words(SQ_ROW_SPLIT, nt) * sizeof(int32_t), s), "set_diffnet_stack(memset)");
    const int extra = (4 * nt + 8 <= p.n_cu && a.L > 1) ? 8 : 0;
    const int nofence = 1;
    hipLaunchKernelGGL(diffnet_stack_split_x2_kernel, dim3(4 * nt + extra), dim3(256), ldsz, s, a, tiles, nt, piece_bytes, stack_fault_tile(),
                       nofence);
    return set_check_launch("set_diffnet_stack");
}

extern "C" int64_t set_diffnet_layer_x3_image_size(int32_t mode) {
    return mode == 2 ? x_nimg<SplitF16x2>() : (mode == 3 ? x_nimg<SplitBf16x3>() : -1);
}

extern "C" int set_pack_diffnet_layer_x3(const float *w_dil, const float *w_out, void *img, int32_t mode, int32_t k1, int32_t k2,
                                         void *stream) {
    SET_REQUIRE(w_dil && w_out && img && (mode == 2 || mode == 3), "set_pack_diffnet_layer_x3");
    SET_REQUIRE(k1 >= -60 && k1 <= 60 && k2 >= -60 && k2 <= 60, "set_pack_diffnet_layer_x3(scale exponents)");
    const float s1 = ldexpf(1.0f, k1), s2 = ldexpf(1.0f, k2);
    unsigned short *im = reinterpret_cast<unsigned short *>(img);
    if (mode == 2)
        hipLaunchKernelGGL(pack_layer_x3_kernel<SplitF16x2>, dim3(set_blocks((x_nimg<SplitF16x2>() - 16) / 2, 256)), dim3(256), 0,
                           (hipStream_t)stream, w_dil, w_out, im, s1, s2);
    else
        hipLaunchKernelGGL(pack_layer_x3_kernel<SplitBf16x3>, dim3(set_blocks((x_nimg<SplitBf16x3>() - 8) / 3, 256)), dim3(256), 0,
                           (hipStream_t)stream, w_dil, w_out, im, s1, s2);
    return set_check_launch("set_pack_diffnet_layer_x3");
}

int set_launch_diffnet_stack_x3(const SetDiffnetStackArgs &a, const StackPlan &p, hipStream_t s) {
    if (p.x3_wino) return p.x3_ncb == 3 ? launch_x3v<3>(a, p.n_cu, s) : launch_x3v<2>(a, p.n_cu, s);
    if (p.family == STACK_X3_F16)
        return p.x3_ncb == 1 ? launch_x3<SplitF16x2, 1, 1>(a, p.n_cu, s) : launch_x3<SplitF16x2, 1, 2>(a, p.n_cu, s);
    return p.x3_ncb == 1 ? launch_x3<SplitBf16x3, 1, 1>(a, p.n_cu, s) : launch_x3<SplitBf16x3, 1, 2>(a, p.n_cu, s);
}
```

### speech-editing-toolkit_amd/csrc/diffusion_loop.hip

```cpp
#include <stdlib.h>

#include "common.h"
#include "diffnet_host.h"
#include "loop_events.h"
#include "stack_queue.h"

namespace {

constexpr int DC = 256;

bool env_int(const char *name, int *v) {
    const char *e = getenv(name);
    if (e) *v = atoi(e);
    return e != nullptr;
}

StackPlan plan_stack(int B, int T, int dcl, bool have_wino, bool have_split, int x3_mode, bool aligned8, int n_cu) {
    StackPlan p = {};
    p.n_cu = n_cu;
    int v = 0, wino_env = 0;
    const bool wino_set = env_int("SET_AMD_WINO", &wino_env);
    const bool f32_pinned = env_int("SET_AMD_SPLIT_F32", &v) && v != 0;
    const bool have_x3 = x3_mode == 2 || x3_mode == 3;
    const int64_t tiles64 = (int64_t)B * ((T + 63) / 64);
    const int64_t split_blocks = 4 * (int64_t)B * ((T + 31) / 32);
    const bool split_one_per_cu = have_x3 && !f32_pinned;
    const bool split_fits = have_split && dcl <= 4 && split_blocks <= (split_one_per_cu ? 1 : 2) * (int64_t)n_cu;
    const bool split_pays = split_blocks <= (int64_t)(have_x3 ? 1 : 2) * n_cu;
    int split_env = 1;
    (void)env_int("SET_AMD_SPLIT", &split_env);
    if (split_fits && (split_env == 2 || (split_env == 1 && !wino_set && split_pays))) {
        p.family = STACK_ROW_SPLIT;
        p.split_x2 = x3_mode == 2 && !f32_pinned;
        return p;
    }
    int x3_env = 1;
    (void)env_int("SET_AMD_X3", &x3_env);
    if (have_x3 && dcl <= 4 && (x3_env == 2 || (x3_env == 1 && !wino_set && tiles64 >= 8))) {
        p.family = x3_mode == 3 ? STACK_X3_BF16 : STACK_X3_F16;
        bool narrow = 5 * tiles64 < 3 * (int64_t)n_cu;
        if (env_int("SET_AMD_X3_TILE", &v)) narrow = v == 32;
        p.x3_ncb = narrow ? 1 : 2;
        int wino = 1;
        (void)env_int("SET_AMD_X3_WINO", &wino);
        if (x3_mode == 2 && dcl == 1 && T % 2 == 0 && !narrow && wino > 0 && aligned8) {
            const int64_t tiles96 = ((int64_t)B * ((T + 31) / 32) + 2) / 3;
            p.x3_wino = true;
            p.x3_ncb = wino == 2 || wino == 3 ? wino : (tiles96 >= (int64_t)n_cu ? 3 : 2);
        }
        return p;
    }
    int ncb = tiles64 < 3 * n_cu ? 1 : 2;
    if (env_int("SET_AMD_STACK_NCB", &v)) ncb = v == 2 ? 2 : 1;
    const bool wino_ok = have_wino && (1 << (dcl - 1)) <= STACK_WINO_MAX_DIL;
    bool wino = wino_ok && 25 * tiles64 >= 17 * n_cu;
    if (wino_set) wino = wino_ok && (wino_env == 2 || (wino && wino_env != 0));
    p.family = wino ? STACK_WINO : (ncb == 1 ? STACK_DIRECT32 : STACK_DIRECT64);
    return p;
}

StackPlan plan_stack_of_images(int B, int T, int dcl, int images) {
    int n_cu = 256;
    (void)set_cu_count(&n_cu);
    return plan_stack(B, T, dcl, (images & 1) != 0, (images & 2) != 0, (images & 4) ? 3 : ((images & 8) ? 2 : 0), true, n_cu);
}

StackPlan stack_plan(const SetDiffnetStackArgs &a, int n_cu) {
    const bool plain = !a.x_all && !a.save_y && !a.save_z;
    const bool aligned8 = ((reinterpret_cast<uintptr_t>(a.condproj) | reinterpret_cast<uintptr_t>(a.xa) | reinterpret_cast<uintptr_t>(a.xb)) & 7) == 0 &&
                          ((a.cp_bs | a.cp_ls) & 1) == 0;
    return plan_stack(a.B, a.T, a.dilation_cycle_length, a.w1w_all && a.w2w_all, a.w1s_all && a.w2s_all && a.z_ws && plain,
                      (a.wx3_all && plain) ? a.x3_mode : 0, aligned8, n_cu);
}

int stack_validate(const SetDiffnetStackArgs &a) {
    SET_REQUIRE(a.xa && a.xb && a.skip && a.condproj && a.dstep && a.w1p_all && a.w2p_all && a.b_dil_all &&
                    a.b_out_all && a.sync_ws,
                "set_diffnet_stack");
    SET_REQUIRE(a.B > 0 && a.T > 0 && a.L > 0 && a.dilation_cycle_length >= 1 && a.dilation_cycle_length <= 4,
                "set_diffnet_stack");
    return SET_OK;
}

int stack_launch(const SetDiffnetStackArgs &a, const StackPlan &p, hipStream_t s) {
    if (p.family >= STACK_X3_BF16) return set_launch_diffnet_stack_x3(a, p, s);
    if (p.split_x2) return set_launch_diffnet_stack_split_x2(a, p, s);
    return set_launch_diffnet_stack_f32(a, p, s);
}

}

extern "C" int set_diffnet_stack(const SetDiffnetStackArgs *args, void *stream) {
    SET_REQUIRE(args != nullptr, "set_diffnet_stack");
    if (int rc = stack_validate(*args)) return rc;
    int n_cu = 0;
    SET_HIP(set_cu_count(&n_cu), "set_diffnet_stack");
    return stack_launch(*args, stack_plan(*args, n_cu), (hipStream_t)stream);
}
extern "C" int set_diffnet_stack_variant(int B, int T, int dilation_cycle_length, int images) {
    return plan_stack_of_images(B, T, dilation_cycle_length, images).family;
}
extern "C" int set_diffnet_stack_x3_winograd(int B, int T, int dilation_cycle_length, int images) {
    const StackPlan p = plan_stack_of_images(B, T, dilation_cycle_length, images);
    return p.family == STACK_X3_F16 && p.x3_wino ? p.x3_ncb : 0;
}

namespace {

SetConv1dArgs conv1x1_args(const float *in, const float *wp, const float *bias, float *out, int B, int Cin, int Cout, int T) {
    SetConv1dArgs c = {};
    c.in = in; c.w = wp; c.bias = bias; c.out = out;
    c.in_bs = (int64_t)Cin * T; c.in_cs = T; c.out_bs = (int64_t)Cout * T; c.out_cs = T;
    c.B = B; c.Cin = Cin; c.Cout = Cout; c.K = 1; c.dil = 1; c.pad = 0;
    c.T_in = T; c.T_iter = T; c.T_out = T; c.out_stride = 1; c.out_off = 0;
    c.alpha = 1.0f; c.impl = SET_IMPL_MFMA;
    return c;
}

hipStream_t g_aux_streams[8] = {nullptr};
int aux_stream(int i, hipStream_t *out) {
    if (!g_aux_streams[i]) SET_HIP(hipStreamCreateWithFlags(&g_aux_streams[i], hipStreamNonBlocking), "aux stream");
    *out = g_aux_streams[i];
    return SET_OK;
}

enum StepBody {
    STEP_STACK,
    STEP_BF16_GROUPS,
    STEP_BF16_LAYERS,
    STEP_F32_LAYERS,
};
struct StepPlan {
    StepBody body;
    int fuse;
    bool fused_boundary;
    bool boundary_x2;
    StackPlan stack;
};

struct Chain {
    const SetDiffLoopArgs &a;
    int b0, Bg;
    hipStream_t s;
    float *x, *ws_x0, *ws_x1, *ws_skip, *ws_h, *ws_x0pred;
    const float *condproj;
    StepPlan plan;
    SetDiffnetStackArgs stack;
    int64_t bf16_per_utt;
};

int plan_steps(Chain &c, int g) {
    const SetDiffLoopArgs &a = c.a;
    const int T = a.T, L = a.L, dcl = a.dilation_cycle_length;
    StepPlan &p = c.plan;
    int n_cu = 0;
    SET_HIP(set_cu_count(&n_cu), "set_diffusion_loop");
    p.fused_boundary = boundary_fusable(a);
    const bool x2_images = p.fused_boundary && a.w_skip_x2 && a.w_outp_x2 && a.w_in_x2 && a.M <= 96;
    if (a.img16_all) {
        p.fuse = 1;
        if (a.bf16_ws && dcl <= 2) {
            p.fuse = set_diffnet_layers_bf16_plan(c.Bg, T, L, dcl);
            if (env_int("SET_AMD_BF16_FUSE", &p.fuse)) p.fuse = p.fuse < 1 ? 1 : (p.fuse > 16 ? 16 : p.fuse);
            if (p.fuse > 1 && a.bf16_ws_floats < set_diffnet_layers_bf16_scratch_floats(a.B, T, 0, p.fuse, dcl)) p.fuse = 1;
        }
        p.body = p.fuse > 1 ? STEP_BF16_GROUPS : STEP_BF16_LAYERS;
        if (p.fuse > 1) c.bf16_per_utt = set_diffnet_layers_bf16_scratch_floats(1, T, 0, p.fuse, dcl);
        p.boundary_x2 = x2_images;
    } else if (a.persistent) {
        p.body = STEP_STACK;
        SetDiffnetStackArgs &sa = c.stack;
        sa.xa = c.ws_x0; sa.xb = c.ws_x1; sa.skip = c.ws_skip;
        sa.condproj = c.condproj; sa.cp_bs = (int64_t)L * 512 * T; sa.cp_ls = (int64_t)512 * T;
        sa.dstep = a.dstep; sa.d_bs = 0; sa.d_cs = a.steps; sa.d_ls = (int64_t)DC * a.steps;
        sa.w1p_all = a.w1p_all; sa.w2p_all = a.w2p_all; sa.b_dil_all = a.b_dil_all; sa.b_out_all = a.b_out_all;
        sa.w1w_all = a.w1w_all; sa.w2w_all = a.w2w_all;
        sa.w1s_all = a.w1s_all; sa.w2s_all = a.w2s_all; sa.wx3_all = a.wx3_all; sa.x3_mode = a.x3_mode;
        sa.z_ws = a.z_ws ? a.z_ws + (int64_t)c.b0 * DC * 32 * ((T + 31) / 32) : nullptr;
        sa.err_flag = a.err_flag;
        sa.sync_ws = a.sync_ws ? a.sync_ws + SQ_GROUP_WORDS * (int64_t)g + 2 * (int64_t)c.b0 * ((T + 31) / 32) : nullptr;
        sa.B = c.Bg; sa.T = T; sa.L = L; sa.dilation_cycle_length = dcl;
        if (int rc = stack_validate(sa)) return rc;
        p.stack = stack_plan(sa, n_cu);
        p.boundary_x2 = x2_images && p.stack.two_piece_fp16();
    } else {
        p.body = STEP_F32_LAYERS;
    }
    int v = 0;
    if (env_int("SET_AMD_BOUNDARY_X2", &v)) p.boundary_x2 = p.boundary_x2 && v != 0;
    return SET_OK;
}

int step_stack(const Chain &c, int sid) {
    SetDiffnetStackArgs sa = c.stack;
    sa.dstep += sid;
    return stack_launch(sa, c.plan.stack, c.s);
}

template <typename Launch> int for_layers(const Chain &c, int stride, Launch launch) {
    float *cur = c.ws_x0, *nxt = c.ws_x1;
    int rc = SET_OK;
    for (int l = 0; l < c.a.L && rc == SET_OK; l += stride) {
        rc = launch(l, cur, nxt);
        float *tmp = cur; cur = nxt; nxt = tmp;
    }
    return rc;
}

int step_bf16_groups(const Chain &c, int sid) {
    const SetDiffLoopArgs &a = c.a;
    const int L = a.L, fuse = c.plan.fuse;
    return for_layers(c, fuse, [&](int l, float *cur, float *nxt) {
        SetDiffnetLayersBf16Args fa = {};
        fa.x_in = cur; fa.x_out = nxt; fa.skip = c.ws_skip;
        fa.cond = a.cond + (int64_t)c.b0 * 192 * a.T;
        fa.dstep = a.dstep + sid; fa.d_bs = 0; fa.d_cs = a.steps; fa.d_ls = (int64_t)DC * a.steps;
        fa.img = reinterpret_cast<const uint16_t *>(a.img16_all) + (int64_t)l * set_diffnet_layer_bf16_image_size();
        fa.b_dil = a.b_dil_all + (int64_t)l * 512; fa.b_cond = a.b_cond_all + (int64_t)l * 512; fa.b_out = a.b_out_all + (int64_t)l * 512;
        fa.scratch = a.bf16_ws + (int64_t)c.b0 * c.bf16_per_utt; fa.scratch_floats = (int64_t)c.Bg * c.bf16_per_utt;
        fa.B = c.Bg; fa.T = a.T; fa.l0 = l; fa.nl = L - l < fuse ? L - l : fuse; fa.dilation_cycle_length = a.dilation_cycle_length;
        fa.first = (l == 0);
        return set_diffnet_layers_fwd_bf16(&fa, c.s);
    });
}

int step_bf16_layers(const Chain &c, int sid) {
    const SetDiffLoopArgs &a = c.a;
    return for_layers(c, 1, [&](int l, float *cur, float *nxt) {
        SetDiffnetLayerBf16Args la = {};
        la.x_in = cur; la.x_out = nxt; la.skip = c.ws_skip;
        la.cond = a.cond + (int64_t)c.b0 * 192 * a.T;
        la.dstep = a.dstep + (int64_t)l * DC * a.steps + sid;
        la.d_bs = 0; la.d_cs = a.steps;
        la.img = reinterpret_cast<const uint16_t *>(a.img16_all) + (int64_t)l * set_diffnet_layer_bf16_image_size();
        la.b_dil = a.b_dil_all + (int64_t)l * 512; la.b_cond = a.b_cond_all + (int64_t)l * 512;
        la.b_out = a.b_out_all + (int64_t)l * 512;
        la.B = c.Bg; la.T = a.T; la.dil = 1 << (l % a.dilation_cycle_length); la.first = (l == 0);
        return set_diffnet_layer_fwd_bf16(&la, c.s);
    });
}

int step_f32_layers(const Chain &c, int sid) {
    const SetDiffLoopArgs &a = c.a;
    return for_layers(c, 1, [&](int l, float *cur, float *nxt) {
        SetDiffnetLayerArgs la = {};
        la.x_in = cur; la.x_out = nxt; la.skip = c.ws_skip;
        la.condproj = c.condproj + (int64_t)l * 512 * a.T;
        la.cp_bs = (int64_t)a.L * 512 * a.T;
        la.dstep = a.dstep + (int64_t)l * DC * a.steps + sid;
        la.d_bs = 0; la.d_cs = a.steps;
        la.w1p = a.w1p_all + (int64_t)l * (512 * 768); la.b_dil = a.b_dil_all + (int64_t)l * 512;
        la.w2p = a.w2p_all + (int64_t)l * (512 * 256); la.b_out = a.b_out_all + (int64_t)l * 512;
        la.B = c.Bg; la.T = a.T; la.dil = 1 << (l % a.dilation_cycle_length); la.first = (l == 0);
        return set_diffnet_layer(&la, c.s);
    });
}

int diffusion_chain(const SetDiffLoopArgs &a, int g, int b0, int Bg, hipStream_t s, hipEvent_t *ev) {
    const int T = a.T, M = a.M, L = a.L;
    const int64_t per_batch = (int64_t)M * T;
    Chain c = {a, b0, Bg, s};
    c.x = a.x + (int64_t)b0 * per_batch;
    c.ws_x0 = a.ws_x0 + (int64_t)b0 * DC * T; c.ws_x1 = a.ws_x1 + (int64_t)b0 * DC * T;
    c.ws_skip = a.ws_skip + (int64_t)b0 * DC * T; c.ws_h = a.ws_h + (int64_t)b0 * DC * T;
    c.ws_x0pred = a.ws_x0pred + (int64_t)b0 * per_batch;
    c.condproj = a.condproj ? a.condproj + (int64_t)b0 * L * 512 * T : nullptr;
    if (int rc = plan_steps(c, g)) return rc;
    const StepPlan &p = c.plan;
    const uint64_t quads_before = (uint64_t)((int64_t)b0 * per_batch / 4);
    const uint64_t quads_total = (uint64_t)(((int64_t)a.B * per_batch + 3) / 4);
    int rc = SET_OK;
    for (int k = 0; k < a.steps && rc == SET_OK; ++k) {
        const int sid = a.steps - 1 - k;
        if (!p.fused_boundary || k == 0) {
            SetConv1dArgs cin = conv1x1_args(c.x, a.w_in_p, a.b_in, c.ws_x0, Bg, M, DC, T);
            cin.act = SET_ACT_RELU;
            rc = set_conv1d(&cin, s);
            if (rc != SET_OK) break;
        }
        if (ev) (void)hipEventRecord(ev[2 * k], s);
        switch (p.body) {
            case STEP_STACK: rc = step_stack(c, sid); break;
            case STEP_BF16_GROUPS: rc = step_bf16_groups(c, sid); break;
            case STEP_BF16_LAYERS: rc = step_bf16_layers(c, sid); break;
            case STEP_F32_LAYERS: rc = step_f32_layers(c, sid); break;
        }
        if (ev) (void)hipEventRecord(ev[2 * k + 1], s);
        if (rc != SET_OK) break;
        const float *eps = a.noise ? a.noise + (int64_t)k * a.B * per_batch + (int64_t)b0 * per_batch : nullptr;
        const uint64_t quad_offset = (uint64_t)(k + 1) * quads_total + quads_before;
        if (p.fused_boundary) {
            rc = launch_boundary(a, Bg, c.ws_skip, c.x, eps, sid, quad_offset, k + 1 < a.steps ? c.ws_x0 : nullptr, p.boundary_x2, s);
            continue;
        }
        SetConv1dArgs cs = conv1x1_args(c.ws_skip, a.w_skip_p, a.b_skip, c.ws_h, Bg, DC, DC, T);
        cs.pro = SET_PRO_DIV; cs.pro_param = sqrtf((float)L); cs.act = SET_ACT_RELU;
        rc = set_conv1d(&cs, s);
        if (rc != SET_OK) break;
        SetConv1dArgs co = conv1x1_args(c.ws_h, a.w_outp_p, a.b_outp, c.ws_x0pred, Bg, DC, M, T);
        rc = set_conv1d(&co, s);
        if (rc != SET_OK) break;
        rc = set_posterior_step(c.ws_x0pred, c.x, eps, a.coef4 + 4 * sid, 0, c.x, Bg, per_batch, a.seed, quad_offset, s);
    }
    return rc;
}

}

extern "C" int set_diffusion_loop(const SetDiffLoopArgs *args, void *stream) {
    SET_REQUIRE(args != nullptr, "set_diffusion_loop");
    const SetDiffLoopArgs &a = *args;
    SET_REQUIRE(a.B > 0 && a.T > 0 && a.M > 0 && a.L > 0 && a.steps > 0 && a.dilation_cycle_length >= 1,
                "set_diffusion_loop");
    SET_REQUIRE(a.x && a.dstep && a.coef4 && a.w_in_p && a.b_in && a.b_dil_all && a.b_out_all && a.w_skip_p && a.b_skip &&
                    a.w_outp_p && a.b_outp, "set_diffusion_loop");
    if (a.img16_all) {
        SET_REQUIRE(a.cond && a.b_cond_all, "set_diffusion_loop(bf16 loop needs cond and b_cond_all)");
    } else {
        SET_REQUIRE(a.condproj && a.w1p_all && a.w2p_all, "set_diffusion_loop");
        SET_REQUIRE(!a.persistent || a.sync_ws, "set_diffusion_loop(persistent needs sync_ws)");
    }
    SET_REQUIRE(a.ws_x0 && a.ws_x1 && a.ws_skip && a.ws_h && a.ws_x0pred, "set_diffusion_loop");
    hipStream_t s = (hipStream_t)stream;
    const int64_t per_batch = (int64_t)a.M * a.T;
    int G = a.n_groups < 1 ? 1 : (a.n_groups > 8 ? 8 : a.n_groups);
    if (G > a.B) G = a.B;
    if (per_batch % 4 != 0) G = 1;
    const bool timing = a.layer_span_ms != nullptr;
    LoopEvents events;
    std::vector<hipEvent_t> ev(timing ? (size_t)2 * a.steps * G : 0);
    for (hipEvent_t &e : ev) SET_HIP(events.create(&e, true), "set_diffusion_loop(event)");
    hipEvent_t loop_ev[2] = {nullptr, nullptr};
    if (a.loop_ms) {
        SET_HIP(events.create(&loop_ev[0], true), "set_diffusion_loop(event)");
        SET_HIP(events.create(&loop_ev[1], true), "set_diffusion_loop(event)");
        (void)hipEventRecord(loop_ev[0], s);
    }
    int rc = SET_OK;
    if (G == 1) {
        rc = diffusion_chain(a, 0, 0, a.B, s, timing ? ev.data() : nullptr);
    } else {
        hipEvent_t fork = nullptr, join = nullptr;
        SET_HIP(events.create(&fork, false), "set_diffusion_loop(fork)");
        SET_HIP(hipEventRecord(fork, s), "set_diffusion_loop(fork)");
        for (int g = 0; g < G && rc == SET_OK; ++g) {
            const int b0 = (int)((int64_t)a.B * g / G), b1 = (int)((int64_t)a.B * (g + 1) / G);
            hipStream_t sg;
            rc = aux_stream(g, &sg);
            if (rc != SET_OK) break;
            SET_HIP(hipStreamWaitEvent(sg, fork, 0), "set_diffusion_loop(fork wait)");
            rc = diffusion_chain(a, g, b0, b1 - b0, sg, timing ? ev.data() + (size_t)2 * a.steps * g : nullptr);
            SET_HIP(events.create(&join, false), "set_diffusion_loop(join)");
            SET_HIP(hipEventRecord(join, sg), "set_diffusion_loop(join)");
            SET_HIP(hipStreamWaitEvent(s, join, 0), "set_diffusion_loop(join wait)");
        }
    }
    if (a.loop_ms) (void)hipEventRecord(loop_ev[1], s);
    if (timing || a.loop_ms) {
        if (rc == SET_OK) {
            hipError_t e = hipStreamSynchronize(s);
            if (e != hipSuccess) rc = set_fail(SET_E_LAUNCH, "set_diffusion_loop(sync)", hipGetErrorString(e));
        }
        if (rc == SET_OK && timing) {
            for (int k = 0; k < a.steps; ++k) {
                float acc_ms = 0.0f;
                for (int g = 0; g < G; ++g) {
                    float ms = 0.0f;
                    (void)hipEventElapsedTime(&ms, ev[(size_t)2 * a.steps * g + 2 * k], ev[(size_t)2 * a.steps * g + 2 * k + 1]);
                    acc_ms += ms;
                }
                a.layer_span_ms[k] = acc_ms / (float)G;
            }
        }
        if (rc == SET_OK && a.loop_ms) (void)hipEventElapsedTime(a.loop_ms, loop_ev[0], loop_ev[1]);
    }
    return rc;
}

extern "C" int64_t set_sizeof_diff_loop_args(void) { return (int64_t)sizeof(SetDiffLoopArgs); }
```

### speech-editing-toolkit_amd/ops.py

```python
import collections
import ctypes as C
import math
import os
import typing

import torch

from . import _lib
from ._lib import (ACT, PRO, IMPL_BF16, IMPL_MFMA, IMPL_MFMA2, IMPL_NAIVE, SetConv1dArgs, SetDiffnetLayerArgs,
                   SetDiffLoopArgs, SetDiffnetStackArgs, check)

_DEFAULT_IMPL = os.environ.get("SET_AMD_CONV_IMPL", "auto")
_WEIGHTS_EPOCH = 0


_COMPUTE_DTYPE = os.environ.get("SET_AMD_DTYPE", "f32")


def set_compute_dtype(dtype):
    global _COMPUTE_DTYPE
    if dtype not in ("f32", "bf16"):
        raise ValueError("compute dtype must be 'f32' or 'bf16', got %r" % (dtype,))
    _COMPUTE_DTYPE = dtype

# ... 1073 lines not shown
    w1w: typing.Optional[torch.Tensor] = None
    w2w: typing.Optional[torch.Tensor] = None
    w1s: typing.Optional[torch.Tensor] = None
    w2s: typing.Optional[torch.Tensor] = None
    wx3: typing.Optional[SplitOperandImages] = None


def _set_images(a, images, B, T, dcl, dev):
    if not isinstance(images, StackImages):
        raise TypeError("the layer stack takes its weight images as an ops.StackImages (fields by name), not %s: a bare tuple in the "
                        "wrong order would launch on the wrong image" % type(images).__name__)
    a.w1p_all, a.w2p_all = images.w1p.data_ptr(), images.w2p.data_ptr()
    a.b_dil_all, a.b_out_all = images.b_dil.data_ptr(), images.b_out.data_ptr()
    if images.w1w is not None:
        a.w1w_all, a.w2w_all = images.w1w.data_ptr(), images.w2w.data_ptr()
    x3 = images.wx3
    if x3 is not None:
        a.wx3_all, a.x3_mode = x3.data.data_ptr(), x3.mode
    if images.w1s is None or stack_variant(B, T, dcl, x3_mode=x3.mode if x3 is not None else 0) != 3:
        return None
    a.w1s_all, a.w2s_all = images.w1s.data_ptr(), images.w2s.data_ptr()
    z_ws = torch.empty(B * ((T + 31) // 32) * 256 * 32, dtype=torch.float32, device=dev)
    a.z_ws = z_ws.data_ptr()
    return z_ws


def diffnet_stack(xa, xb, skip, condproj, dstep_ptr, d_bs, d_cs, d_ls, images, dilation_cycle_length, sync_ws=None,
                  x_all=None, save_y=None, save_z=None, err_flag=None):
    B, Cc, T = xa.shape
    assert Cc == 256
    a = SetDiffnetStackArgs()
    z_ws = _set_images(a, images, B, T, dilation_cycle_length, xa.device)
    _f(xa), _f(xb), _f(skip), _f(condproj)
    L = images.b_dil.shape[0]
    if sync_ws is None:
        sync_ws = torch.empty(sync_ws_size(B, T), dtype=torch.int32, device=xa.device)
    a.xa, a.xb, a.skip = xa.data_ptr(), xb.data_ptr(), skip.data_ptr()
    a.condproj, a.dstep = condproj.data_ptr(), dstep_ptr
    if x_all is not None:
        a.x_all, a.save_y, a.save_z = _f(x_all).data_ptr(), _f(save_y).data_ptr(), _f(save_z).data_ptr()
    if err_flag is not None:
        a.err_flag = err_flag.data_ptr()
    a.sync_ws = sync_ws.data_ptr()
    a.cp_bs, a.cp_ls = condproj.stride(0), 512 * T
    a.d_bs, a.d_cs, a.d_ls = int(d_bs), int(d_cs), int(d_ls)
    a.B, a.T, a.L, a.dilation_cycle_length = B, T, L, int(dilation_cycle_length)
    check(_lib.lib().set_diffnet_stack(C.byref(a), _stream()), "set_diffnet_stack")
    return sync_ws


def diffnet_layer(x_in, condproj, cp_bs, dstep, d_bs, d_cs, w1p, b_dil, w2p, b_out, x_out, skip, dil, first,
                  dbg_clock=None):
    _f(x_in), _f(x_out), _f(skip)
    B, Cc, T = x_in.shape
    assert Cc == 256
    a = SetDiffnetLayerArgs()
    a.x_in, a.condproj, a.dstep = x_in.data_ptr(), condproj, dstep
    a.w1p, a.b_dil, a.w2p, a.b_out = w1p.data_ptr(), b_dil.data_ptr(), w2p.data_ptr(), b_out.data_ptr()
    a.x_out, a.skip = x_out.data_ptr(), skip.data_ptr()
    a.cp_bs, a.d_bs, a.d_cs = int(cp_bs), int(d_bs), int(d_cs)
    a.B, a.T, a.dil, a.first = B, T, int(dil), int(bool(first))
    a.dbg_clock = dbg_clock.data_ptr() if dbg_clock is not None else None
    check(_lib.lib().set_diffnet_layer(C.byref(a), _stream()), "set_diffnet_layer")


def posterior_step(x0, x_t, coef4, eps=None, out=None, seed=0, offset=0):
    _f(x0), _f(x_t), _f(coef4), _f(eps)
    B = x0.shape[0]
    per_batch = x0.numel() // B
    out = x_t if out is None else out
    assert coef4.shape[0] in (1, B) and coef4.shape[-1] == 4
    coef_bs = 0 if coef4.shape[0] == 1 else 4
    check(_lib.lib().set_posterior_step(_p(x0), _p(x_t), _p(eps), _p(coef4), coef_bs, _p(out), B, per_batch, int(seed),
                                        int(offset), _stream()), "set_posterior_step")
    return out


def q_sample(x_start, eps, ab2, nonpad=None):
    _f(x_start), _f(eps), _f(ab2), _f(nonpad)
    B, M, T = x_start.shape[0], x_start.shape[-2], x_start.shape[-1]
    out = torch.empty_like(x_start)
    check(_lib.lib().set_q_sample(_p(x_start), _p(eps), _p(ab2), _p(nonpad), _p(out), B, M, T, _stream()),
          "set_q_sample")
    return out


def randn(shape, device, seed=0, offset=0):
    out = torch.empty(shape, dtype=torch.float32, device=device)
    check(_lib.lib().set_randn(_p(out), out.numel(), int(seed), int(offset), _stream()), "set_randn")
    return out


def fanout(x, n):
    return (x,) * n


def grad_scale(x, s):
    return x


def dropout(x, p, seed, offset=0):
    return x


def res_skip_fn(x, o, skip_in):
    first = skip_in is None
    skip = torch.empty_like(x) if first else skip_in
    return res_skip(x, o, skip, first), skip


def selftest_mfma():
    err = C.c_float(-1.0)
    check(_lib.lib().set_selftest_mfma(C.byref(err), _stream()), "set_selftest_mfma")
    return float(err.value)


def diffusion_loop(*, x, noise, seed, condproj, dstep, coef4, w_in, b_in, packs, w_skip, b_skip,
                   w_outp, b_outp, L, steps, dilation_cycle_length, want_layer_spans=False, n_groups=None,
                   persistent=None, bf16=None):
    _f(x), _f(noise), _f(condproj), _f(dstep), _f(coef4)
    B, M, T = x.shape
    dev = x.device
    ws = [torch.empty(B, 256, T, dtype=torch.float32, device=dev) for _ in range(4)]
    ws_x0pred = torch.empty(B, M, T, dtype=torch.float32, device=dev)
    a = SetDiffLoopArgs()
    a.B, a.T, a.M, a.L, a.steps, a.dilation_cycle_length = B, T, M, L, steps, dilation_cycle_length
    a.x = x.data_ptr()
    a.noise = noise.data_ptr() if noise is not None else None
    a.seed = int(seed)
    a.condproj = condproj.data_ptr() if condproj is not None else None
    a.dstep, a.coef4 = dstep.data_ptr(), coef4.data_ptr()
    if bf16 is not None:
        a.cond, a.img16_all, a.b_cond_all = _f(bf16["cond"]).data_ptr(), bf16["imgs"].data_ptr(), _f(bf16["b_cond"]).data_ptr()
        n_ws = max(_lib.lib().set_diffnet_layers_bf16_scratch_floats(B, T, 0, n, dilation_cycle_length) for n in range(2, 17)) \
            if dilation_cycle_length <= 2 else 0
        if n_ws > 0:
            bf16_ws = torch.empty(n_ws, dtype=torch.float32, device=dev)
            a.bf16_ws, a.bf16_ws_floats = bf16_ws.data_ptr(), n_ws
    a.w_in_p, a.b_in = w_in.packed().data_ptr(), b_in.data_ptr()
    z_ws = _set_images(a, packs, B, T, dilation_cycle_length, dev)
    a.persistent = int(default_persistent() if persistent is None else bool(persistent))
    sync_ws = torch.empty(sync_ws_size(B, T), dtype=torch.int32, device=dev)
    a.sync_ws = sync_ws.data_ptr()
    err = torch.zeros(1, dtype=torch.int32, device=dev)
    a.err_flag = err.data_ptr()
    bf16_bx2 = bf16 is not None and split_operand_mode() == 2
    use_bx2 = ((a.wx3_all and a.x3_mode == 2) or bf16_bx2) and M <= 96 and os.environ.get("SET_AMD_BOUNDARY_X2", "1") != "0"
    if use_bx2:
        a.w_skip_x2, a.w_outp_x2, a.w_in_x2 = (w.packed_x2().data_ptr() for w in (w_skip, w_outp, w_in))
    a.w_skip_p, a.b_skip = w_skip.packed().data_ptr(), b_skip.data_ptr()
    a.w_outp_p, a.b_outp = w_outp.packed().data_ptr(), b_outp.data_ptr()
    a.ws_x0, a.ws_x1, a.ws_skip, a.ws_h = (w.data_ptr() for w in ws)
    a.ws_x0pred = ws_x0pred.data_ptr()
    a.n_groups = default_groups(B, T) if n_groups is None else int(n_groups)
    spans, loop_ms = None, None
    if want_layer_spans:
        spans = (C.c_float * steps)()
        a.layer_span_ms = C.cast(spans, C.POINTER(C.c_float))
        loop_ms = C.c_float(0.0)
        a.loop_ms = C.pointer(loop_ms)
    check(_lib.lib().set_diffusion_loop(C.byref(a), _stream()), "set_diffusion_loop")
    if a.persistent or use_bx2:
        code = int(err.item())
        if code == 2:
            raise SplitRangeError("set_diffusion_loop: an activation of magnitude >= 32768 is outside the range of the fp16 "
                                  "operand splitting; set SET_AMD_SPLIT_OPERAND=bf16x3 (fp32 range) or SET_AMD_X3=0")
        if code != 0:
            raise _lib.SetAmdError("set_diffusion_loop: a tile dependency wait of the persistent layer-stack kernel timed out")
    if spans is None:
        return None
    return {"layer_span_ms": list(spans), "loop_ms": float(loop_ms.value), "n_groups": int(a.n_groups),
            "persistent": int(a.persistent)}


def default_persistent():
    return os.environ.get("SET_AMD_PERSISTENT", "1") != "0"


def default_groups(B, T):
    return 1


class MatView:

    def __init__(self, tensor, n_outer, n_inner, rows, cols, bo_s, bi_s, rs, cs, offset=0):
        self.tensor = _f(tensor)
        self.n_outer, self.n_inner, self.rows, self.cols = int(n_outer), int(n_inner), int(rows), int(cols)
        self.bo_s, self.bi_s, self.rs, self.cs, self.offset = int(bo_s), int(bi_s), int(rs), int(cs), int(offset)

    @property
    def t(self):
        return MatView(self.tensor, self.n_outer, self.n_inner, self.cols, self.rows, self.bo_s, self.bi_s, self.cs,
                       self.rs, self.offset)

    @staticmethod
    def heads(x, heads, chan0=0, width=None):
        B, Ctot, T = x.shape
        H = Ctot - chan0 if width is None else width
        d = H // heads
        assert x.is_contiguous() and d * heads == H and chan0 + H <= Ctot
        return MatView(x, B, heads, T, d, Ctot * T, d * T, 1, T, offset=chan0 * T)

    @staticmethod
    def scores(s):
        B, h, Tq, Tk = s.shape
        assert s.is_contiguous()
        return MatView(s, B, h, Tq, Tk, h * Tq * Tk, Tq * Tk, Tk, 1)

    def ptr(self):
        return self.tensor.data_ptr() + 4 * self.offset


def bmm(a, b, c, alpha=1.0, accumulate=False):
    assert a.cols == b.rows and a.rows == c.rows and b.cols == c.cols
    assert (a.n_outer, a.n_inner) == (b.n_outer, b.n_inner) == (c.n_outer, c.n_inner)
    if c.rs == 1 and c.cs != 1:
        a, b, c = b.t, a.t, c.t
    g = _lib.SetBmmArgs()
    g.A, g.B, g.C = a.ptr(), b.ptr(), c.ptr()
    g.a_bo, g.a_bi, g.a_ms, g.a_ks = a.bo_s, a.bi_s, a.rs, a.cs
    g.b_bo, g.b_bi, g.b_ks, g.b_ns = b.bo_s, b.bi_s, b.rs, b.cs
    g.c_bo, g.c_bi, g.c_ms, g.c_ns = c.bo_s, c.bi_s, c.rs, c.cs
    g.n_outer, g.n_inner, g.M, g.N, g.K = c.n_outer, c.n_inner, c.rows, c.cols, a.cols
    g.alpha, g.accumulate = float(alpha), int(bool(accumulate))
    check(_lib.lib().set_bmm(C.byref(g), _stream()), "set_bmm")
    return c.tensor


def softmax_rows(x, key_padding_mask=None, rows_per_batch=1, fill=float("-inf"), out=None):
    _f(x), _f(key_padding_mask)
    cols = x.shape[-1]
    rows = x.numel() // cols
    out = torch.empty_like(x) if out is None else out
    check(_lib.lib().set_softmax_rows(_p(x), _p(key_padding_mask), _p(out), rows, cols, int(rows_per_batch), float(fill),
                                      _stream()), "set_softmax_rows")
    return out


def softmax_rows_bwd(p, dp):
    _f(p), _f(dp)
    cols = p.shape[-1]
    ds = torch.empty_like(p)
    check(_lib.lib().set_softmax_rows_bwd(_p(p), _p(dp), _p(ds), p.numel() // cols, cols, _stream()), "set_softmax_rows_bwd")
    return ds


def make_positions(tokens=None, x_bct=None):
    if tokens is not None:
        _i(tokens)
        B, T = tokens.shape
        pos = torch.empty(B, T, dtype=torch.int64, device=tokens.device)
        check(_lib.lib().set_make_positions(_p(tokens), None, 0, _p(pos), B, T, _stream()), "set_make_positions")
    else:
        _f(x_bct)
        B, Cc, T = x_bct.shape
        pos = torch.empty(B, T, dtype=torch.int64, device=x_bct.device)
        check(_lib.lib().set_make_positions(None, _p(x_bct), Cc * T, _p(pos), B, T, _stream()), "set_make_positions")
    return pos


def head_mean(p):
    _f(p)
    B, h = p.shape[:2]
    out = torch.empty((B,) + tuple(p.shape[2:]), dtype=torch.float32, device=p.device)
    check(_lib.lib().set_head_mean(_p(p), _p(out), B, h, out.numel() // B, _stream()), "set_head_mean")
    return out


def mask_fill_chan(x, e, m):
    _f(x), _f(e), _f(m)
    B, Cc, T = x.shape
    out = torch.empty_like(x)
    check(_lib.lib().set_mask_fill_chan(_p(x), _p(e), _p(m), _p(out), B, Cc, T, _stream()), "set_mask_fill_chan")
    return out


def masked_channel_sum(d, m, out):
    _f(d), _f(m), _f(out)
    B, Cc, T = d.shape
    check(_lib.lib().set_masked_channel_sum(_p(d), _p(m), _p(out), B, Cc, T, _stream()), "set_masked_channel_sum")
    return out


def attention_fused_on(head_dim=None):
    if head_dim is not None and int(head_dim) not in (32, 64, 96):
        return False
    return os.environ.get("SET_AMD_ATTN_FUSED", "1") != "0"


def _attn_args(qv, kv, vv, o, lse, heads, key_padding_mask, fill, alpha, p=None):
    d = qv.cols
    assert qv.rs == 1 and kv.rs == 1 and vv.rs == 1 and kv.cols == d and vv.cols == d and kv.rows == vv.rows
    assert qv.bi_s == d * qv.cs and kv.bi_s == d * kv.cs and vv.bi_s == d * vv.cs
    a = _lib.SetAttnArgs()
    a.q, a.k, a.v = qv.ptr(), kv.ptr(), vv.ptr()
    a.o, a.lse = o.data_ptr(), lse.data_ptr()
    a.p = p.data_ptr() if p is not None else None
    a.kpm = _f(key_padding_mask, "key_padding_mask").data_ptr() if key_padding_mask is not None else None
    a.q_bs, a.k_bs, a.v_bs, a.o_bs = qv.bo_s, kv.bo_s, vv.bo_s, o.stride(0)
    a.q_cs, a.k_cs, a.v_cs, a.o_cs = qv.cs, kv.cs, vv.cs, o.stride(1)
    a.B, a.heads, a.head_dim, a.Tq, a.Tk = qv.n_outer, heads, d, qv.rows, kv.rows
    a.scale, a.fill = float(alpha), float(fill)
    a.bf16 = int(_COMPUTE_DTYPE == "bf16")
    return a


# ... 60 lines not shown
```

Baseline: 174,300.

## Store diffnet workspace activations in channel-quad layout for 128-bit buffer accesses

Adds a channel-quad (4 channels interleaved per time step) layout for the x/skip workspaces used by the Winograd split-operand stack kernel and the fused x2 boundary kernel. Loads and stores become 128-bit buffer operations instead of scalar per-channel accesses. A relayout kernel converts the first step's input conv output, and the boundary kernel writes the next step's input directly in quad layout. It is enabled by default when alignment and plan conditions hold, at the cost of an extra relayout launch on the first step and s_nop padding after each wide store.

```diff
diff --git a/include/set_amd.h b/include/set_amd.h
--- a/include/set_amd.h
+++ b/include/set_amd.h
@@ -172,6 +172,7 @@
     float *z_ws;
     const void *wx3_all;
     int32_t x3_mode;
+    int32_t xs_q4;
 } SetDiffnetStackArgs;
 int set_diffnet_stack(const SetDiffnetStackArgs *args, void *stream);
 int64_t set_sizeof_diffnet_stack_args(void);
@@ -234,6 +235,7 @@
     const float *b_cond_all;
     float *bf16_ws;
     int64_t bf16_ws_floats;
+    int32_t ws_q4;
 } SetDiffLoopArgs;
 int set_diffusion_loop(const SetDiffLoopArgs *args, void *stream);
 
diff --git a/speech-editing-toolkit_amd/_lib.py b/speech-editing-toolkit_amd/_lib.py
--- a/speech-editing-toolkit_amd/_lib.py
+++ b/speech-editing-toolkit_amd/_lib.py
@@ -73,6 +73,7 @@
         ("err_flag", C.c_void_p),
         ("cond", C.c_void_p), ("img16_all", C.c_void_p), ("b_cond_all", C.c_void_p),
         ("bf16_ws", C.c_void_p), ("bf16_ws_floats", C.c_int64),
+        ("ws_q4", C.c_int32),
     ]
 
 
@@ -87,7 +88,7 @@
         ("x_all", C.c_void_p), ("save_y", C.c_void_p), ("save_z", C.c_void_p),
         ("err_flag", C.c_void_p),
         ("w1s_all", C.c_void_p), ("w2s_all", C.c_void_p), ("z_ws", C.c_void_p), ("wx3_all", C.c_void_p),
-        ("x3_mode", C.c_int32),
+        ("x3_mode", C.c_int32), ("xs_q4", C.c_int32),
     ]
 
 
diff --git a/speech-editing-toolkit_amd/csrc/boundary.hip b/speech-editing-toolkit_amd/csrc/boundary.hip
--- a/speech-editing-toolkit_amd/csrc/boundary.hip
+++ b/speech-editing-toolkit_amd/csrc/boundary.hip
@@ -160,6 +160,7 @@
     int32_t *err_flag;
 };
 
+template <bool Q4>
 __global__ void __launch_bounds__(256, 2) diffnet_boundary_x2_kernel(BoundaryX2Args ax) {
     const BoundaryArgs &a = ax.g;
     extern __shared__ __attribute__((aligned(16))) unsigned char bl[];
@@ -173,12 +174,21 @@
     {
         const int f = lane, cg = w;
         const rsrc_t rs = make_rsrc(a.skip + (int64_t)b * DC * T);
-        const unsigned vo = 4u * (unsigned)min(t0 + f, T - 1);
+        const unsigned vo = (Q4 ? 16u : 4u) * (unsigned)min(t0 + f, T - 1);
         const bool tv = t0 + f < T;
         for (int c0 = 0; c0 < 64; c0 += 16) {
             float v[16];
-#pragma unroll
-            for (int u = 0; u < 16; ++u) v[u] = buf_load(rs, vo, (unsigned)(64 * cg + c0 + u) * T4);
+            if (Q4) {
+#pragma unroll
+                for (int j = 0; j < 4; ++j) {
+                    const f32x4 q = buf_load4(rs, vo, (unsigned)(64 * cg + c0 + 4 * j) * T4);
+#pragma unroll
+                    for (int e = 0; e < 4; ++e) v[4 * j + e] = q[e];
+                }
+            } else {
+#pragma unroll
+                for (int u = 0; u < 16; ++u) v[u] = buf_load(rs, vo, (unsigned)(64 * cg + c0 + u) * T4);
+            }
 #pragma unroll
             for (int q8 = 0; q8 < 2; ++q8) {
                 u32x4_t u0, u1;
@@ -336,14 +346,25 @@
 #pragma unroll
         for (int cb = 0; cb < 2; ++cb) {
             if (t0 + 32 * cb + l31 < T) {
-                const unsigned so = 4u * (unsigned)(4 * half * T + t0 + 32 * cb + l31);
-#pragma unroll
-                for (int i = 0; i < 2; ++i)
+                const unsigned so = Q4 ? 16u * (unsigned)(half * T + t0 + 32 * cb + l31) : 4u * (unsigned)(4 * half * T + t0 + 32 * cb + l31);
+#pragma unroll
+                for (int i = 0; i < 2; ++i) {
+                    if (Q4) {
+#pragma unroll
+                        for (int j = 0; j < 4; ++j) {
+                            f32x4 q;
+#pragma unroll
+                            for (int e = 0; e < 4; ++e) q[e] = fmaxf(acc[i][cb][4 * j + e] * inv + bin[i][4 * j + e], 0.0f);
+                            buf_store4_padded<false>(q, ro, so, (unsigned)(32 * (2 * w + i) + 8 * j) * T4);
+                        }
+                        continue;
+                    }
 #pragma unroll
                     for (int r = 0; r < 16; ++r) {
                         const int ur = 32 * (2 * w + i) + urow16(r);
                         buf_store(fmaxf(acc[i][cb][r] * inv + bin[i][r], 0.0f), ro, so, 4u * (unsigned)ur * (unsigned)T);
                     }
+                }
             }
         }
     }
@@ -355,10 +376,32 @@
     return a.T % 4 == 0 && a.M <= 96 && a.M >= 2 && ((a.M + 15) / 16 * 16 / 2) % 8 == 0;
 }
 
+__global__ void __launch_bounds__(256) relayout_q4_kernel(const float *src, float *dst, int T, int64_t n_quads) {
+    const int64_t i = (int64_t)blockIdx.x * 256 + threadIdx.x;
+    if (i >= n_quads) return;
+    const int64_t bq = i / T;
+    const int t = (int)(i - bq * T);
+    const float *p = src + bq * 4 * T + t;
+    f32x4 v;
+#pragma unroll
+    for (int e = 0; e < 4; ++e) v[e] = p[(int64_t)e * T];
+    *reinterpret_cast<f32x4 *>(dst + 4 * i) = v;
+}
+
+int launch_relayout_q4(const float *src, float *dst, int Bg, int T, hipStream_t s) {
+    const int64_t n_quads = (int64_t)Bg * (DC / 4) * T;
+    SET_REQUIRE((n_quads + 255) / 256 < ((int64_t)1 << 31), "set_diffusion_loop(relayout)");
+    hipLaunchKernelGGL(relayout_q4_kernel, dim3((unsigned)((n_quads + 255) / 256)), dim3(256), 0, s, src, dst, T, n_quads);
+    return set_check_launch("set_diffusion_loop(relayout)");
+}
+
 int launch_boundary(const SetDiffLoopArgs &a, int Bg, const float *skip, float *x, const float *eps, int sid, uint64_t quad_offset,
-                    float *xin_next, bool x2, hipStream_t s) {
+                    float *xin_next, bool x2, bool q4, hipStream_t s) {
     static SetDeviceOnce lds_once;
-    if (int rc = set_lds_optin(lds_once, 80 * 1024, "boundary(attr)", diffnet_boundary_kernel, diffnet_boundary_x2_kernel)) return rc;
+    if (int rc = set_lds_optin(lds_once, 80 * 1024, "boundary(attr)", diffnet_boundary_kernel, diffnet_boundary_x2_kernel<false>,
+                               diffnet_boundary_x2_kernel<true>))
+        return rc;
+    SET_REQUIRE(!q4 || x2, "set_diffusion_loop(boundary: the channel-quad layout needs the two-piece fp16 boundary)");
     BoundaryArgs g = {};
     g.skip = skip; g.x = x; g.eps = eps; g.coef4 = a.coef4 + 4 * sid;
     g.w_skip_p = a.w_skip_p; g.b_skip = a.b_skip; g.w_outp_p = a.w_outp_p; g.b_outp = a.b_outp;
@@ -372,7 +415,10 @@
         gx.w_outp_x2 = reinterpret_cast<const unsigned short *>(a.w_outp_x2);
         gx.w_in_x2 = reinterpret_cast<const unsigned short *>(a.w_in_x2);
         gx.err_flag = a.err_flag;
-        hipLaunchKernelGGL(diffnet_boundary_x2_kernel, dim3((a.T + 63) / 64, Bg), dim3(256), (size_t)2 * BX_PIECE, s, gx);
+        if (q4)
+            hipLaunchKernelGGL(diffnet_boundary_x2_kernel<true>, dim3((a.T + 63) / 64, Bg), dim3(256), (size_t)2 * BX_PIECE, s, gx);
+        else
+            hipLaunchKernelGGL(diffnet_boundary_x2_kernel<false>, dim3((a.T + 63) / 64, Bg), dim3(256), (size_t)2 * BX_PIECE, s, gx);
     } else {
         hipLaunchKernelGGL(diffnet_boundary_kernel, dim3((a.T + 63) / 64, Bg), dim3(256), (size_t)DC * BD_LD * sizeof(float), s, g);
     }
diff --git a/speech-editing-toolkit_amd/csrc/common.h b/speech-editing-toolkit_amd/csrc/common.h
--- a/speech-editing-toolkit_amd/csrc/common.h
+++ b/speech-editing-toolkit_amd/csrc/common.h
@@ -173,6 +173,14 @@
 __device__ __forceinline__ void buf_store_agent(float v, rsrc_t r, unsigned voff, unsigned soff) {
     __builtin_amdgcn_raw_buffer_store_b32(__builtin_bit_cast(unsigned, v), r, (int)voff, (int)soff, 16);
 }
+__host__ __device__ inline int64_t q4f_index(int c, int t, int T) { return ((int64_t)(c >> 2) * T + t) * 4 + (c & 3); }
+template <bool AGENT>
+__device__ __forceinline__ void buf_store4_padded(f32x4 v, rsrc_t r, unsigned voff, unsigned soff) {
+    __builtin_amdgcn_raw_buffer_store_b128(__builtin_bit_cast(u32x4_t, v), r, (int)voff, (int)soff, AGENT ? 16 : 0);
+    __builtin_amdgcn_sched_barrier(0);
+    asm volatile("s_nop 1" ::: "memory");
+    __builtin_amdgcn_sched_barrier(0);
+}
 
 __device__ __forceinline__ void split2_f16(float a, float b, unsigned &p0, unsigned &p1) {
     typedef _Float16 h2_t __attribute__((ext_vector_type(2)));
diff --git a/speech-editing-toolkit_amd/csrc/diffnet_host.h b/speech-editing-toolkit_amd/csrc/diffnet_host.h
--- a/speech-editing-toolkit_amd/csrc/diffnet_host.h
+++ b/speech-editing-toolkit_amd/csrc/diffnet_host.h
@@ -26,4 +26,5 @@
 
 bool boundary_fusable(const SetDiffLoopArgs &a);
 int launch_boundary(const SetDiffLoopArgs &a, int Bg, const float *skip, float *x, const float *eps, int sid, uint64_t quad_offset,
-                    float *xin_next, bool x2, hipStream_t s);
+                    float *xin_next, bool x2, bool q4, hipStream_t s);
+int launch_relayout_q4(const float *src, float *dst, int Bg, int T, hipStream_t s);
diff --git a/speech-editing-toolkit_amd/csrc/diffnet_x3.hip b/speech-editing-toolkit_amd/csrc/diffnet_x3.hip
--- a/speech-editing-toolkit_amd/csrc/diffnet_x3.hip
+++ b/speech-editing-toolkit_amd/csrc/diffnet_x3.hip
@@ -566,8 +566,8 @@
     }
 }
 
-template <int NB, int PH>
-__device__ __forceinline__ void x3v_stage_load(const X3Tile &a, int w, int lane, f32x2 (&x12)[NB][8], float (&xh)[NB][8]) {
+template <int NB, int PH, bool Q4>
+__device__ __forceinline__ void x3v_stage_load(const X3Tile &a, int w, int lane, float (&xs)[NB][16], float (&xh)[NB][8]) {
     const int l15 = lane & 15, cs = lane >> 4;
     const int ch0 = 32 * w + 8 * cs;
     const int T = a.T;
@@ -578,11 +578,36 @@
         const X3Col c = x3_col(a, nb);
         const rsrc_t rx = make_rsrc(a.xin + (int64_t)c.b * XC * T);
         const int t = c.t0 + 2 * l15;
+        const int th = l15 == 0 ? c.t0 - 1 : c.t0 + 32;
+        if (Q4) {
+            const unsigned vox = 16u * (unsigned)(2 * cs * T + min(t, T - 2)), soff = (unsigned)(32 * w) * T4;
+#pragma unroll
+            for (int q = 0; q < 2; ++q)
+#pragma unroll
+                for (int f = 0; f < 2; ++f) {
+                    const f32x4 v = buf_load4(rx, vox + 16u * (unsigned)f, soff + (unsigned)(4 * q) * T4);
+#pragma unroll
+                    for (int i = 0; i < 4; ++i) xs[nb][2 * (4 * q + i) + f] = v[i];
+                }
+            if (PH == 1 && edge) {
+                const unsigned voh = 16u * (unsigned)(2 * cs * T + min(max(th, 0), T - 1));
+#pragma unroll
+                for (int q = 0; q < 2; ++q) {
+                    const f32x4 v = buf_load4(rx, voh, soff + (unsigned)(4 * q) * T4);
+#pragma unroll
+                    for (int i = 0; i < 4; ++i) xh[nb][4 * q + i] = v[i];
+                }
+            }
+            continue;
+        }
         const unsigned vox = 4u * (unsigned)min(t, T - 2) + (unsigned)ch0 * T4;
 #pragma unroll
-        for (int k = 0; k < 8; ++k) x12[nb][k] = buf_load2(rx, vox, (unsigned)k * T4);
+        for (int k = 0; k < 8; ++k) {
+            const f32x2 v = buf_load2(rx, vox, (unsigned)k * T4);
+            xs[nb][2 * k] = v[0];
+            xs[nb][2 * k + 1] = v[1];
+        }
         if (PH == 1) {
-            const int th = l15 == 0 ? c.t0 - 1 : c.t0 + 32;
             const unsigned voh = 4u * (unsigned)min(max(th, 0), T - 1) + (unsigned)ch0 * T4;
             if (edge) {
 #pragma unroll
@@ -592,7 +617,7 @@
     }
 }
 template <int NB, int PH>
-__device__ __forceinline__ float x3v_stage_store(const X3Tile &a, unsigned char *lds, const float *dsh, int w, int lane, const f32x2 (&x12)[NB][8],
+__device__ __forceinline__ float x3v_stage_store(const X3Tile &a, unsigned char *lds, const float *dsh, int w, int lane, const float (&xs)[NB][16],
                                                  const float (&xh)[NB][8]) {
     typedef SplitF16x2 S;
     const int l15 = lane & 15, cs = lane >> 4;
@@ -615,7 +640,7 @@
             for (int h = 0; h < 2; ++h) {
                 const int e = 2 * e2 + h;
                 const float ds = e < 4 ? dA[e & 3] : dB[e & 3];
-                const float d1 = v12 ? x12[nb][e][0] + ds : 0.0f, d2 = v12 ? x12[nb][e][1] + ds : 0.0f;
+                const float d1 = v12 ? xs[nb][2 * e] + ds : 0.0f, d2 = v12 ? xs[nb][2 * e + 1] + ds : 0.0f;
                 if (PH == 0) {
                     V[0][h] = d1 + d2;
                     V[1][h] = d2 - d1;
@@ -678,7 +703,37 @@
     }
 }
 
-template <int NB>
+template <bool Q4, bool NT>
+__device__ __forceinline__ void x3v_rows_load(float (&v)[16], rsrc_t r, unsigned voff, int w, unsigned T4) {
+    if (Q4) {
+#pragma unroll
+        for (int j = 0; j < 4; ++j) {
+            const f32x4 q = NT ? buf_load4_stream(r, voff, (unsigned)(32 * w + 8 * j) * T4) : buf_load4(r, voff, (unsigned)(32 * w + 8 * j) * T4);
+#pragma unroll
+            for (int i = 0; i < 4; ++i) v[4 * j + i] = q[i];
+        }
+    } else {
+#pragma unroll
+        for (int k = 0; k < 16; ++k) v[k] = NT ? buf_load_nt(r, voff, (unsigned)(32 * w + urow16(k)) * T4) : buf_load(r, voff, (unsigned)(32 * w + urow16(k)) * T4);
+    }
+}
+template <bool Q4>
+__device__ __forceinline__ void x3v_rows_store(const float (&v)[16], rsrc_t r, unsigned voff, int w, unsigned T4) {
+    if (Q4) {
+#pragma unroll
+        for (int j = 0; j < 4; ++j) {
+            f32x4 q;
+#pragma unroll
+            for (int i = 0; i < 4; ++i) q[i] = v[4 * j + i];
+            buf_store4_padded<true>(q, r, voff, (unsigned)(32 * w + 8 * j) * T4);
+        }
+    } else {
+#pragma unroll
+        for (int k = 0; k < 16; ++k) buf_store_agent(v[k], r, voff, (unsigned)(32 * w + urow16(k)) * T4);
+    }
+}
+
+template <int NB, bool Q4>
 __device__ __forceinline__ void x3v_main(const X3Tile &a, f32x4 (&PQ)[2][4][NB], unsigned char *lds, PhaseProbe<11> &pp, PhaseTimeline<32> &tl) {
     pp.lap(0); tl.mark(8);
     typedef SplitF16x2 S;
@@ -701,10 +756,10 @@
     const unsigned abase = (unsigned)((x_n1<S>() + x_n2<S>() + 8) * 2) + (unsigned)(w * X_KSV * 4 * 2 * 1024);
     const unsigned boff = (unsigned)(l15 * XRV + kg * 16);
     u32x4_t A[PFV][4][2];
-    f32x2 x12[NB][8];
+    float xs[NB][16];
     float xh[NB][8];
-    x3v_stage_load<NB, 0>(a, w, lane, x12, xh);
-    float amax = x3v_stage_store<NB, 0>(a, lds, dsh, w, lane, x12, xh);
+    x3v_stage_load<NB, 0, Q4>(a, w, lane, xs, xh);
+    float amax = x3v_stage_store<NB, 0>(a, lds, dsh, w, lane, xs, xh);
 #pragma unroll
     for (int p = 0; p < PFV; ++p)
 #pragma unroll
@@ -717,7 +772,7 @@
     x3v_plane<NB, PFV>(PQ[0], A, rw, lane16, abase, 0, lds, boff);
     x3v_plane<NB, PFV>(PQ[1], A, rw, lane16, abase, 1, lds + xv_plane<NB>(), boff);
     pp.lap(2); tl.mark(10);
-    x3v_stage_load<NB, 1>(a, w, lane, x12, xh);
+    x3v_stage_load<NB, 1, Q4>(a, w, lane, xs, xh);
     __builtin_amdgcn_sched_barrier(0);
 #pragma unroll
     for (int mb = 0; mb < 4; ++mb)
@@ -731,7 +786,7 @@
             }
     __syncthreads();
     tl.mark(21);
-    amax = fmaxf(amax, x3v_stage_store<NB, 1>(a, lds, dsh, w, lane, x12, xh));
+    amax = fmaxf(amax, x3v_stage_store<NB, 1>(a, lds, dsh, w, lane, xs, xh));
     if (!(amax < 32768.0f) && a.err_flag) __hip_atomic_store(a.err_flag, 2, __ATOMIC_RELAXED, __HIP_MEMORY_SCOPE_AGENT);
 #pragma unroll
     for (int p = 0; p < PFV; ++p)
@@ -753,15 +808,14 @@
         const X3Col c = x3_col(a, cb);
         const int t = c.t0 + l31;
         tv[cb] = c.ok && t < T;
-        vo4[cb] = 4u * (unsigned)(4 * half * T + min(t, T - 1));
+        vo4[cb] = Q4 ? 16u * (unsigned)(half * T + min(t, T - 1)) : 4u * (unsigned)(4 * half * T + min(t, T - 1));
         ub[cb] = (int64_t)c.b * XC * T;
     }
     float xres[NB][16];
 #pragma unroll
     for (int cb = 0; cb < NB; ++cb) {
         const rsrc_t rx = make_rsrc(a.xin + ub[cb]);
-#pragma unroll
-        for (int r = 0; r < 16; ++r) xres[cb][r] = buf_load(rx, vo4[cb], (unsigned)(32 * w + urow16(r)) * T4);
+        x3v_rows_load<Q4, false>(xres[cb], rx, vo4[cb], w, T4);
     }
     __syncthreads();
     tl.mark(23);
@@ -818,16 +872,17 @@
 #pragma unroll
         for (int cb = 0; cb < NB; ++cb) {
             const rsrc_t rsk = make_rsrc(a.skp + ub[cb]);
-#pragma unroll
-            for (int r = 0; r < 16; ++r) sk[cb][r] = buf_load_nt(rsk, vo4[cb], (unsigned)(32 * w + urow16(r)) * T4);
+            x3v_rows_load<Q4, true>(sk[cb], rsk, vo4[cb], w, T4);
         }
     }
 #pragma unroll
     for (int cb = 0; cb < NB; ++cb) {
         if (tv[cb]) {
             const rsrc_t rxo = make_rsrc(a.xout + ub[cb]);
-#pragma unroll
-            for (int r = 0; r < 16; ++r) buf_store_agent((acc[0][0][cb][r] * is2) * RSQRT2, rxo, vo4[cb], (unsigned)(32 * w + urow16(r)) * T4);
+            float o[16];
+#pragma unroll
+            for (int r = 0; r < 16; ++r) o[r] = (acc[0][0][cb][r] * is2) * RSQRT2;
+            x3v_rows_store<Q4>(o, rxo, vo4[cb], w, T4);
         }
     }
     tl.mark(25);
@@ -835,9 +890,10 @@
     for (int cb = 0; cb < NB; ++cb) {
         if (tv[cb]) {
             const rsrc_t rsk = make_rsrc(a.skp + ub[cb]);
-#pragma unroll
-            for (int r = 0; r < 16; ++r)
-                buf_store_agent(first ? acc[0][1][cb][r] * is2 : acc[0][1][cb][r] * is2 + sk[cb][r], rsk, vo4[cb], (unsigned)(32 * w + urow16(r)) * T4);
+            float o[16];
+#pragma unroll
+            for (int r = 0; r < 16; ++r) o[r] = first ? acc[0][1][cb][r] * is2 : acc[0][1][cb][r] * is2 + sk[cb][r];
+            x3v_rows_store<Q4>(o, rsk, vo4[cb], w, T4);
         }
     }
     pp.lap(10); tl.mark(18);
@@ -846,7 +902,7 @@
 #ifndef X3V_TL_TASK
 #define X3V_TL_TASK 10
 #endif
-template <int NB>
+template <int NB, bool Q4>
 __global__ void __launch_bounds__(512, 1) diffnet_stack_x3v_kernel(SetDiffnetStackArgs a, int ntiles, int ntasks, int fault_tile) {
     typedef SplitF16x2 S;
     extern __shared__ __attribute__((aligned(16))) unsigned char lds[];
@@ -912,7 +968,7 @@
         }
         const int n_next = __builtin_amdgcn_readfirstlane(s_task[0]);
         tl.mark(4);
-        x3v_main<NB>(lt, PQ, lds, pp, tl);
+        x3v_main<NB, Q4>(lt, PQ, lds, pp, tl);
 #if SET_PHASE_PROBE == 2
         if (++n_mine == X3V_TL_TASK && (tid == 0 || tid == 448) && g_x3_phase_buf) {
             const rsrc_t rt = make_rsrc(g_x3_phase_buf);
@@ -937,20 +993,22 @@
     pp.flush(g_x3_phase_buf);
 }
 
-template <int NB>
+template <int NB, bool Q4>
 int launch_x3v(const SetDiffnetStackArgs &a, int n_cu, hipStream_t s) {
     static SetDeviceOnce lds_once;
-    if (int rc = set_lds_optin(lds_once, 160 * 1024, "set_diffnet_stack(x3v attr)", diffnet_stack_x3v_kernel<NB>)) return rc;
+    if (int rc = set_lds_optin(lds_once, 160 * 1024, "set_diffnet_stack(x3v attr)", diffnet_stack_x3v_kernel<NB, Q4>)) return rc;
     const int Q = a.B * ((a.T + 31) / 32);
     const int ntiles = (Q + NB - 1) / NB;
     const int64_t ntasks64 = (int64_t)ntiles * a.L;
     SET_REQUIRE(ntasks64 < (1ll << 30), "set_diffnet_stack(task count)");
     SET_REQUIRE((int64_t)2 * XC * a.T * 4 < ((int64_t)1 << 31), "set_diffnet_stack(split-operand kernel: T too large)");
     SET_REQUIRE(a.dilation_cycle_length == 1 && a.T % 2 == 0, "set_diffnet_stack(x3v: dilation 1 and even T only)");
+    SET_REQUIRE(!Q4 || ((reinterpret_cast<uintptr_t>(a.xa) | reinterpret_cast<uintptr_t>(a.xb) | reinterpret_cast<uintptr_t>(a.skip)) & 15) == 0,
+                "set_diffnet_stack(xs_q4: xa, xb and skip must be 16-byte aligned)");
     const size_t ldsz = (size_t)xv_tile<NB>() + NB * XC * sizeof(float) + 16;
     SET_HIP(set_zero_async(a.sync_ws, stack_sync_words(SQ_QUEUE, ntiles) * sizeof(int32_t), s), "set_diffnet_stack(memset)");
     const int grid = stack_grid(n_cu, ntiles, ntasks64, NB == 2, 0);
-    hipLaunchKernelGGL(diffnet_stack_x3v_kernel<NB>, dim3(grid), dim3(512), ldsz, s, a, ntiles, (int)ntasks64, stack_fault_tile());
+    hipLaunchKernelGGL((diffnet_stack_x3v_kernel<NB, Q4>), dim3(grid), dim3(512), ldsz, s, a, ntiles, (int)ntasks64, stack_fault_tile());
     return set_check_launch("set_diffnet_stack");
 }
 
@@ -1246,7 +1304,8 @@
 }
 
 int set_launch_diffnet_stack_x3(const SetDiffnetStackArgs &a, const StackPlan &p, hipStream_t s) {
-    if (p.x3_wino) return p.x3_ncb == 3 ? launch_x3v<3>(a, p.n_cu, s) : launch_x3v<2>(a, p.n_cu, s);
+    if (p.x3_wino && a.xs_q4) return p.x3_ncb == 3 ? launch_x3v<3, true>(a, p.n_cu, s) : launch_x3v<2, true>(a, p.n_cu, s);
+    if (p.x3_wino) return p.x3_ncb == 3 ? launch_x3v<3, false>(a, p.n_cu, s) : launch_x3v<2, false>(a, p.n_cu, s);
     if (p.family == STACK_X3_F16)
         return p.x3_ncb == 1 ? launch_x3<SplitF16x2, 1, 1>(a, p.n_cu, s) : launch_x3<SplitF16x2, 1, 2>(a, p.n_cu, s);
     return p.x3_ncb == 1 ? launch_x3<SplitBf16x3, 1, 1>(a, p.n_cu, s) : launch_x3<SplitBf16x3, 1, 2>(a, p.n_cu, s);
diff --git a/speech-editing-toolkit_amd/csrc/diffusion_loop.hip b/speech-editing-toolkit_amd/csrc/diffusion_loop.hip
--- a/speech-editing-toolkit_amd/csrc/diffusion_loop.hip
+++ b/speech-editing-toolkit_amd/csrc/diffusion_loop.hip
@@ -83,6 +83,7 @@
 }
 
 int stack_launch(const SetDiffnetStackArgs &a, const StackPlan &p, hipStream_t s) {
+    SET_REQUIRE(!a.xs_q4 || p.x3_wino, "set_diffnet_stack(xs_q4: only the Winograd split-operand kernel reads the channel-quad layout)");
     if (p.family >= STACK_X3_BF16) return set_launch_diffnet_stack_x3(a, p, s);
     if (p.split_x2) return set_launch_diffnet_stack_split_x2(a, p, s);
     return set_launch_diffnet_stack_f32(a, p, s);
@@ -135,6 +136,7 @@
     int fuse;
     bool fused_boundary;
     bool boundary_x2;
+    bool ws_q4;
     StackPlan stack;
 };
 
@@ -188,6 +190,11 @@
     }
     int v = 0;
     if (env_int("SET_AMD_BOUNDARY_X2", &v)) p.boundary_x2 = p.boundary_x2 && v != 0;
+    int q4_env = 1;
+    (void)env_int("SET_AMD_WS_Q4", &q4_env);
+    const bool aligned16 = ((reinterpret_cast<uintptr_t>(c.ws_x0) | reinterpret_cast<uintptr_t>(c.ws_x1) | reinterpret_cast<uintptr_t>(c.ws_skip)) & 15) == 0;
+    p.ws_q4 = a.ws_q4 != 0 && q4_env != 0 && p.body == STEP_STACK && p.stack.x3_wino && p.fused_boundary && p.boundary_x2 && aligned16;
+    c.stack.xs_q4 = p.ws_q4 ? 1 : 0;
     return SET_OK;
 }
 
@@ -273,9 +280,10 @@
     for (int k = 0; k < a.steps && rc == SET_OK; ++k) {
         const int sid = a.steps - 1 - k;
         if (!p.fused_boundary || k == 0) {
-            SetConv1dArgs cin = conv1x1_args(c.x, a.w_in_p, a.b_in, c.ws_x0, Bg, M, DC, T);
+            SetConv1dArgs cin = conv1x1_args(c.x, a.w_in_p, a.b_in, p.ws_q4 ? c.ws_x1 : c.ws_x0, Bg, M, DC, T);
             cin.act = SET_ACT_RELU;
             rc = set_conv1d(&cin, s);
+            if (rc == SET_OK && p.ws_q4) rc = launch_relayout_q4(c.ws_x1, c.ws_x0, Bg, T, s);
             if (rc != SET_OK) break;
         }
         if (ev) (void)hipEventRecord(ev[2 * k], s);
@@ -290,7 +298,7 @@
         const float *eps = a.noise ? a.noise + (int64_t)k * a.B * per_batch + (int64_t)b0 * per_batch : nullptr;
         const uint64_t quad_offset = (uint64_t)(k + 1) * quads_total + quads_before;
         if (p.fused_boundary) {
-            rc = launch_boundary(a, Bg, c.ws_skip, c.x, eps, sid, quad_offset, k + 1 < a.steps ? c.ws_x0 : nullptr, p.boundary_x2, s);
+            rc = launch_boundary(a, Bg, c.ws_skip, c.x, eps, sid, quad_offset, k + 1 < a.steps ? c.ws_x0 : nullptr, p.boundary_x2, p.ws_q4, s);
             continue;
         }
         SetConv1dArgs cs = conv1x1_args(c.ws_skip, a.w_skip_p, a.b_skip, c.ws_h, Bg, DC, DC, T);
diff --git a/speech-editing-toolkit_amd/ops.py b/speech-editing-toolkit_amd/ops.py
--- a/speech-editing-toolkit_amd/ops.py
+++ b/speech-editing-toolkit_amd/ops.py
@@ -1249,6 +1249,7 @@
     a.w_outp_p, a.b_outp = w_outp.packed().data_ptr(), b_outp.data_ptr()
     a.ws_x0, a.ws_x1, a.ws_skip, a.ws_h = (w.data_ptr() for w in ws)
     a.ws_x0pred = ws_x0pred.data_ptr()
+    a.ws_q4 = 1
     a.n_groups = default_groups(B, T) if n_groups is None else int(n_groups)
     spans, loop_ms = None, None
     if want_layer_spans:
```

Result: faster. 179,500, median of 6 (+3.0%).
